# RL-VIG/LibContinual

Measured on AMD Instinct MI355X. Metric: images/sec/node (task-0 epoch), CIFAR-100 B50-5x10, higher is better.
Workload: dtype bf16; 1 GPU; lwf_resnet18_b50_task0; method=LWF, backbone=resnet18, per_gpu_batch=256, global_batch=256, image=3x32x32, parallelism=dp1, optimizer=fused SGD

## Files before the change

### include/clhip.h

```cpp
#ifndef CLHIP_H
#define CLHIP_H

#include <stddef.h>
#include <stdint.h>

#ifdef __cplusplus
extern "C" {
#endif

#define CLHIP_OK 0
#define CLHIP_EINVAL (-1)
#define CLHIP_EHIP (-2)
#define CLHIP_ENOMEM (-3)

#define CLHIP_BF16 0
#define CLHIP_F32 1

const char* clhip_last_error(void);
int clhip_version(void);

int clhip_nchw_to_nhwc(const float* x, void* y, int N, int C, int H, int W, int Cpad, int dtype, void* stream);
int clhip_nhwc_to_nchw(const void* y, float* x, int N, int C, int H, int W, int dtype, void* stream);

int clhip_conv_weight_prep(const float* w, void* w_fwd, void* w_dg, int K, int taps, int Creal, int Cpad,
// ... 19 lines not shown
                     int stride, int pad, int dtype, void* stream);

int clhip_bn_stats_finalize(const float* stat_partials, int tiles, int64_t M, int C, const float* gamma, const float* beta,
                            float* running_mean, float* running_var, float momentum, float eps, float* mean,
                            float* invstd, float* scale, float* shift, void* stream);
int clhip_bn_eval_affine(const float* gamma, const float* beta, const float* running_mean, const float* running_var,
                         float eps, int C, float* scale, float* shift, void* stream);
int clhip_bn_apply(const void* z, const float* scale, const float* shift, const void* res, void* y, int64_t M, int C,
                   int relu, int dtype, void* stream);
int clhip_bn_apply_eval(const void* z, const float* gamma, const float* beta, const float* running_mean, const float* running_var, float eps,
                        const void* res , void* y, int64_t M, int C, int relu, int dtype, void* stream);
int clhip_bn_apply_train(const void* z, const double* stat_acc, int replicas, int64_t M, int C, const float* gamma, const float* beta, float* rm,
                         float* rv, float momentum, float eps, float* mean, float* invstd, const void* res , void* y,
                         int relu, int dtype, void* stream);
int clhip_bn_apply_train_mask(const void* z, const double* stat_acc, int replicas, int64_t M, int C, const float* gamma, const float* beta, float* rm,
                              float* rv, float momentum, float eps, float* mean, float* invstd, const void* res , void* y,
                              void* relu_mask, int dtype, void* stream);
int clhip_bn_bwd_acc(const void* dy, const void* y, const void* z, const float* mean, const float* invstd, const float* gamma,
                     float* dgamma, float* dbeta, void* dz, void* dres, int dres_accumulate, int64_t M, int C, int relu, double* acc,
                     int replicas, int dtype, void* stream);
int clhip_bn_bwd_acc_zmask(const void* dy, const void* z, const float* mean, const float* invstd, const float* gamma, const float* beta,
                           float* dgamma, float* dbeta, void* dz, int64_t M, int C, double* acc, int replicas, int dtype, void* stream);
int clhip_bn_bwd_apply_acc(const void* dy, const void* y , const void* z, const float* mean, const float* invstd, const float* gamma,
                           const float* beta , float* dgamma, float* dbeta, void* dz, void* dres , int dres_accumulate,
                           int64_t M, int C, int relu, const double* acc, int replicas, int dtype, void* stream);
int clhip_bn_bwd_blocks(int64_t M, int C);
size_t clhip_bn_bwd_ws_floats(int64_t M, int C);
int clhip_bn_bwd(const void* dy, const void* y, const void* z, const float* mean, const float* invstd, const float* gamma,
                 float* dgamma, float* dbeta, void* dz, void* dres, int dres_accumulate, int64_t M, int C, int relu,
                 float* ws, int dtype, void* stream);

int clhip_avgpool_fwd(const void* a, float* feat, int N, int HW, int C, int dtype, void* stream);
int clhip_avgpool_bwd(const float* dfeat, void* da, int N, int HW, int C, int dtype, void* stream);
int clhip_avgpool_bwd_bn_reduce_supported(int N, int HW, int C, int dtype);
int clhip_avgpool_bwd_bn_reduce(const float* dfeat, void* da, const void* z_prod, const void* y_prod , const float* mean, const float* invstd,
                                double* acc, int replicas, int N, int HW, int C, int dtype, void* stream);

int clhip_maxpool_out_dim(int H);
int clhip_bn_relu_maxpool_fwd(const void* z, const double* stat_acc, int replicas, const float* gamma, const float* beta, float* running_mean,
                              float* running_var, float momentum, float eps, float* mean, float* invstd, void* y, void* argmax , int N, int H,
                              int W, int C, int training, int dtype, void* stream);
int clhip_maxpool_bwd_bn_reduce(const void* dy, const void* argmax, const void* z, const float* mean, const float* invstd, const float* gamma,
                                const float* beta, void* g, double* acc, int replicas, int N, int H, int W, int C, int dtype, void* stream);

int clhip_avgpool_win_fwd(const void* a, float* feat, int N, int H, int W, int C, int win, int dtype, void* stream);
int clhip_avgpool_win_bwd(const float* dfeat, void* da, int N, int H, int W, int C, int win, int dtype, void* stream);

int clhip_add_stats_blocks(int64_t M, int C);
int clhip_add_stats(void* z, const void* r, double* stat_acc, int replicas, int64_t M, int C, int dtype, void* stream);
int clhip_add_inplace(void* a, const void* b, int64_t n, int dtype, void* stream);

enum {
    CLHIP_UNIT_RELU = 1,
    CLHIP_UNIT_PRE_RES = 2,
    CLHIP_UNIT_RAW_SRC = 4,
    CLHIP_UNIT_NO_BN = 8,
    CLHIP_UNIT_MAXPOOL = 16
};

typedef struct {
    int32_t cin, cout, ksize, stride, pad;
    int32_t src;
    int32_t res;
    int32_t relu;
    int64_t w_off;
    int64_t gamma_off;
    int64_t beta_off;
    int64_t rm_off;
    int64_t rv_off;
} clhip_unit_desc;

typedef struct clhip_plan clhip_plan;

clhip_plan* clhip_plan_create(const clhip_unit_desc* units , int n_units, int N, int H, int W, int Cin, int dtype);
clhip_plan* clhip_plan_create_ex(const clhip_unit_desc* units , int n_units, int N, int H, int W, int Cin, int dtype, int pool_win);
void clhip_plan_destroy(clhip_plan*);
size_t clhip_plan_workspace_bytes(const clhip_plan*);
size_t clhip_plan_shadow_bytes(const clhip_plan*);
int clhip_plan_feat_dim(const clhip_plan*);
int clhip_plan_stage_status(clhip_plan*);
long long clhip_plan_stage_info(const clhip_plan*, int what);
int clhip_plan_stage_trace(clhip_plan*, unsigned long long* out24);
int clhip_plan_prep_weights(clhip_plan*, const float* params, void* shadow, void* stream);
int clhip_plan_forward(clhip_plan*, const float* x, const float* params, float* bn_stats, const void* shadow,
                       void* workspace, float* feat, int training, void* stream);
int clhip_plan_forward_ex(clhip_plan*, const float* x, const float* params, float* bn_stats, const void* shadow,
                          void* workspace, float* feat, int training, int64_t* num_batches_tracked, void* stream);
int clhip_plan_backward(clhip_plan*, const float* dfeat, const float* params, const void* shadow, void* workspace,
                        float* grads, void* stream);
int clhip_plan_num_units(const clhip_plan* p);
int clhip_plan_backward_range(clhip_plan* p, const float* dfeat, const float* params, const void* shadow, void* workspace,
                              float* grads, int unit_hi, int unit_lo, void* stream);
int clhip_plan_read_act(clhip_plan*, const void* workspace, int idx, int which, float* out_nchw, void* stream);

int clhip_linear_fwd(const float* x, const float* w, const float* b , float* out, int B, int D, int O, void* stream);
int clhip_linear_bwd(const float* x, const float* w, const float* dout, float* dx , float* dw, float* db ,
                     int B, int D, int O, int accumulate, void* stream);
int clhip_ce_slice(const float* logits, const int64_t* labels, int B, int O, int lo, int hi, int pred_hi, float weight,
                   float* loss_out, int loss_accumulate, float* dlogits , int grad_accumulate,
                   int64_t* pred , int32_t* correct , void* stream);
int clhip_ce_window(const float* logits, const int64_t* labels, int B, int O, int lo, int hi, int pred_lo, int pred_hi, float weight,
                    float* loss_out, int loss_accumulate, float* dlogits , int grad_accumulate,
                    int64_t* pred , int32_t* correct , void* stream);
int clhip_kd_loss(const float* pred, int pred_stride, const float* soft, int soft_stride, int B, int k, float T,
                  float weight, float* loss_out, int loss_accumulate, float* dpred , int grad_accumulate,
                  void* stream);

int clhip_cosine_linear_fwd(const float* x, const float* w, float* out, float* xnorm, float* wnorm, int B, int D, int O, void* stream);
int clhip_cosine_linear_bwd(const float* x, const float* w, const float* out, const float* xnorm, const float* wnorm,
                            const float* dout, float* dx, float* dw, int B, int D, int O, int accumulate, void* stream);
int clhip_cos_embed_loss(const float* a, const float* b, int B, int D, float weight, float* loss_out, int loss_accumulate,
                         float* da, int grad_accumulate, void* stream);
int clhip_margin_rank_loss(const float* scores, const int64_t* labels, int B, int O, int num_old, int K, float margin,
                           float weight, float* loss_out, int loss_accumulate, float* dscores, int grad_accumulate,
                           int32_t* hard_count, void* stream);

int clhip_ewc_penalty(const float* p, const float* ref, const float* fisher, int64_t n, float weight, float* loss_out,
                      int loss_accumulate, void* stream);
int clhip_ewc_grad(const float* p, const float* ref, const float* fisher, float* g, int64_t n, float weight,
                   const float* dev_scale, void* stream);
int clhip_ewc_penalty_multi(int count, const float* const* p, const float* const* ref, const float* const* fisher, const int64_t* n, float weight,
                            float* loss_out, int loss_accumulate, void* stream);
int clhip_ewc_grad_multi(int count, const float* const* p, const float* const* ref, const float* const* fisher, float* const* g, const int64_t* n,
                         float weight, const float* dev_scale, void* stream);
int clhip_fisher_accum(float* fisher, const float* g, int64_t n, float scale, void* stream);
int clhip_fisher_merge(float* new_f, const float* old_f, int64_t n, float alpha, void* stream);
int clhip_sgd_step(float* p, const float* g, float* mom, int64_t n, float lr, float momentum, float weight_decay,
                   float grad_scale, const float* ewc_ref, const float* ewc_fisher, float ewc_weight, void* stream);
int clhip_sgd_step_multi(int count, float* const* p, const float* const* g, float* const* mom , const int64_t* n, float lr, float momentum,
                         float weight_decay, float grad_scale, void* stream);
int clhip_sgd_step_multi_zero(int count, float* const* p, float* const* g, float* const* mom , const int64_t* n, float lr, float momentum,
                              float weight_decay, float grad_scale, unsigned zero_grad_mask, void* stream);
int clhip_adam_step(float* p, const float* g, float* m, float* v, int64_t n, float lr, float beta1, float beta2, float eps,
                    float weight_decay, float grad_scale, int step, void* stream);
int clhip_sq_norm(const float* g, int64_t n, float* out, int accumulate, void* stream);
int clhip_scale(float* g, int64_t n, float s, void* stream);
int clhip_scale_dev(const float* g, float* out, int64_t n, float s, const float* dev_scale, void* stream);
int clhip_sigma_scale_fwd(const float* scores, const float* sigma_dev, float* logits, int64_t n, void* stream);
int clhip_sigma_scale_bwd(const float* scores, const float* sigma_dev, const float* dlogits, float* dscores, float* dsigma,
                          int dsigma_accumulate, int64_t n, void* stream);

int clhip_l2_normalize_rows(const float* x, float* out, int R, int D, void* stream);
int clhip_ncm_classify(const float* feats, const float* means, int B, int M, int D, int64_t* pred, void* stream);
int clhip_herding_select(const float* feats , int n, int D, int m, int32_t* chosen ,
                         float* ws , void* stream);
int clhip_herding_select_batched(const float* feats, const int32_t* offsets, int n_classes, int max_rows, int D, int m, int32_t* chosen, float* ws,
                                 void* stream);

int clhip_gemm_nt(const void* A, const void* B, void* C, const float* bias, const void* R, void* H, int M, int N, int K,
                  int lda, int ldb, int ldc, int ldr, int ldh, int epilogue, int dtype, void* stream);
int clhip_conv_dgrad_wgrad_supported(int N, int H, int W, int C, int Creal, int K, int ksize, int stride, int pad, int dtype);
int clhip_conv_dgrad_wgrad(const void* x, const void* dz, const void* w_dg, void* dx, int accumulate, float* dw, void* ws,
                           const void* z_prod, const void* y_prod, const float* mean, const float* invstd, double* acc, int replicas,
                           int N, int H, int W, int C, int Creal, int K, int ksize, int stride, int pad, int dtype, void* stream);

typedef struct clhip_bn_input {
    const double* stat_acc; int replicas;
    const float* gamma; const float* beta;
    float* running_mean; float* running_var;
    float momentum, eps;
    float* mean; float* invstd;
    float* coef;
} clhip_bn_input;
typedef struct clhip_bn_grad {
    const void* dy; const void* z;
    const double* sums; int replicas;
// ... 119 lines not shown
```

### libcontinual_amd/_lib.py

```python
import ctypes as C
import os
import re
import subprocess

_HERE = os.path.dirname(os.path.abspath(__file__))
LIB_PATH = os.path.join(_HERE, "libclhip.so")
HEADER_PATH = os.path.join(os.path.dirname(_HERE), "include", "clhip.h")

BF16, F32 = 0, 1


class ClhipError(RuntimeError):
    pass


class UnitDesc(C.Structure):
    _fields_ = [("cin", C.c_int32), ("cout", C.c_int32), ("ksize", C.c_int32), ("stride", C.c_int32), ("pad", C.c_int32),
                ("src", C.c_int32), ("res", C.c_int32), ("relu", C.c_int32),
                ("w_off", C.c_int64), ("gamma_off", C.c_int64), ("beta_off", C.c_int64),
                ("rm_off", C.c_int64), ("rv_off", C.c_int64)]


class VitDesc(C.Structure):
    _fields_ = [(n, C.c_int32) for n in ("img", "patch", "dim", "depth", "heads", "mlp", "lora_rank")] + [("block_ln_eps", C.c_float)]
# ... 6 lines not shown

class VitParams(C.Structure):
    _fields_ = [(n, C.c_void_p) for n in ("cls_token", "pos_embed", "pe_w", "pe_b", "norm_w", "norm_b")] + [("layers", C.POINTER(VitLayerParams))]


def build(force=False):
    script = os.path.join(_HERE, "csrc", "build.sh")
    if force:
        import shutil
        shutil.rmtree(os.path.join(_HERE, "csrc", "obj"), ignore_errors=True)
    subprocess.run(["bash", script], check=True)


_lib = None
_p, _i, _l, _f, _sz = C.c_void_p, C.c_int, C.c_int64, C.c_float, C.c_size_t

_PROTOS = {
    "clhip_last_error": (C.c_char_p, []),
    "clhip_version": (_i, []),
    "clhip_nchw_to_nhwc": (_i, [_p, _p, _i, _i, _i, _i, _i, _i, _p]),
    "clhip_nhwc_to_nchw": (_i, [_p, _p, _i, _i, _i, _i, _i, _p]),
    "clhip_conv_weight_prep": (_i, [_p, _p, _p, _i, _i, _i, _i, _i, _p]),
    "clhip_conv_fwd_tiles": (_i, [_i] * 8),
    "clhip_conv_fwd": (_i, [_p, _p, _p, _p] + [_i] * 9 + [_p]),
    "clhip_conv_fwd_acc": (_i, [_p, _p, _p, _p] + [_i] * 10 + [_p]),
    "clhip_bn_apply_train": (_i, [_p, _p, _i, _l, _i, _p, _p, _p, _p, _f, _f, _p, _p, _p, _p, _i, _i, _p]),
    "clhip_bn_apply_train_mask": (_i, [_p, _p, _i, _l, _i, _p, _p, _p, _p, _f, _f, _p, _p, _p, _p, _p, _i, _p]),
    "clhip_bn_bwd_acc": (_i, [_p, _p, _p, _p, _p, _p, _p, _p, _p, _p, _i, _l, _i, _i, _p, _i, _i, _p]),
    "clhip_bn_bwd_acc_zmask": (_i, [_p, _p, _p, _p, _p, _p, _p, _p, _p, _l, _i, _p, _i, _i, _p]),
    "clhip_conv_dgrad": (_i, [_p, _p, _p, _i] + [_i] * 9 + [_p]),
    "clhip_maxpool_out_dim": (_i, [_i]),
    "clhip_bn_relu_maxpool_fwd": (_i, [_p, _p, _i, _p, _p, _p, _p, _f, _f, _p, _p, _p, _p, _i, _i, _i, _i, _i, _i, _p]),
    "clhip_maxpool_bwd_bn_reduce": (_i, [_p, _p, _p, _p, _p, _p, _p, _p, _p, _i, _i, _i, _i, _i, _i, _p]),
    "clhip_conv_dgrad_bn_reduce_supported": (_i, [_i] * 9),
    "clhip_conv_dgrad_bn_reduce": (_i, [_p, _p, _p, _i, _p, _p, _p, _p, _p, _i] + [_i] * 9 + [_p]),
    "clhip_conv_dgrad_bn_reduce_overlapped": (_i, [_i] * 9),
    "clhip_conv_dgrad_bn_reduce_ex": (_i, [_p, _p, _p, _i, _p, _p, _p, _p, _p, _p, _p, _p, _i] + [_i] * 9 + [_p]),
    "clhip_bn_bwd_apply_acc": (_i, [_p, _p, _p, _p, _p, _p, _p, _p, _p, _p, _p, _i, _l, _i, _i, _p, _i, _i, _p]),
    "clhip_conv_wgrad_ws_bytes": (_sz, [_i] * 10),
    "clhip_conv_dgrad_wgrad_supported": (_i, [_i] * 10),
    "clhip_conv_bn_input_supported": (_i, [_i] * 9),
    "clhip_conv_fwd_acc_bn_input": (_i, [_p, _p, _p, _p, _p, _i] + [_i] * 9 + [_p]),
    "clhip_conv_fwd_acc_bn_res_input": (_i, [_p, _p, _p, _p, _p, _p, _i] + [_i] * 9 + [_p]),
    "clhip_conv_dgrad_wgrad_bn_input": (_i, [_p, _p, _p, _p, _p, _i, _p, _p, _p, _p, _p, _i] + [_i] * 10 + [_p]),
    "clhip_conv_dgrad_wgrad_bn_grad": (_i, [_p, _p, _p, _p, _p, _i, _p, _p, _p, _p, _p, _p, _p, _i] + [_i] * 10 + [_p]),
    "clhip_conv_dgrad_pair_supported": (_i, [_i] * 6),
    "clhip_conv_dgrad_pair_packed_bytes": (_sz, [_i, _i]),
    "clhip_conv_dgrad_pair_pack": (_i, [_p, _p, _p, _i, _i, _i, _p]),
    "clhip_conv_dgrad_pair": (_i, [_p, _p, _p, _p, _i] + [_i] * 6 + [_p]),
    "clhip_conv_dgrad_pair_bn_reduce_supported": (_i, [_i] * 6),
    "clhip_conv_dgrad_pair_bn_reduce": (_i, [_p, _p, _p, _p, _i, _p, _p, _p, _p, _p, _i] + [_i] * 6 + [_p]),
    "clhip_conv_wgrad_pair_supported": (_i, [_i] * 6),
    "clhip_conv_fwd_acc_pair_supported": (_i, [_i] * 6),
    "clhip_conv_fwd_acc_pair": (_i, [_p, _p, _p, _p, _p, _p, _i, _p, _i] + [_i] * 6 + [_p]),
    "clhip_conv_wgrad_pair": (_i, [_p] * 7 + [_i] * 6 + [_p]),
    "clhip_conv_dgrad_wgrad": (_i, [_p, _p, _p, _p, _i, _p, _p, _p, _p, _p, _p, _p, _i] + [_i] * 10 + [_p]),
    "clhip_conv_wgrad": (_i, [_p, _p, _p, _p] + [_i] * 10 + [_p]),
    "clhip_bn_stats_finalize": (_i, [_p, _i, _l, _i, _p, _p, _p, _p, _f, _f, _p, _p, _p, _p, _p]),
    "clhip_bn_eval_affine": (_i, [_p, _p, _p, _p, _f, _i, _p, _p, _p]),
    "clhip_bn_apply": (_i, [_p, _p, _p, _p, _p, _l, _i, _i, _i, _p]),
    "clhip_bn_apply_eval": (_i, [_p, _p, _p, _p, _p, _f, _p, _p, _l, _i, _i, _i, _p]),
    "clhip_bn_bwd_blocks": (_i, [_l, _i]),
    "clhip_bn_bwd_ws_floats": (_sz, [_l, _i]),
    "clhip_bn_bwd": (_i, [_p, _p, _p, _p, _p, _p, _p, _p, _p, _p, _i, _l, _i, _i, _p, _i, _p]),
    "clhip_avgpool_fwd": (_i, [_p, _p, _i, _i, _i, _i, _p]),
    "clhip_avgpool_bwd": (_i, [_p, _p, _i, _i, _i, _i, _p]),
    "clhip_avgpool_bwd_bn_reduce_supported": (_i, [_i] * 4),
    "clhip_avgpool_bwd_bn_reduce": (_i, [_p, _p, _p, _p, _p, _p, _p, _i, _i, _i, _i, _i, _p]),
    "clhip_avgpool_win_fwd": (_i, [_p, _p, _i, _i, _i, _i, _i, _i, _p]),
    "clhip_avgpool_win_bwd": (_i, [_p, _p, _i, _i, _i, _i, _i, _i, _p]),
    "clhip_add_stats_blocks": (_i, [_l, _i]),
    "clhip_add_stats": (_i, [_p, _p, _p, _i, _l, _i, _i, _p]),
    "clhip_add_inplace": (_i, [_p, _p, _l, _i, _p]),
    "clhip_plan_create": (_p, [C.POINTER(UnitDesc), _i, _i, _i, _i, _i, _i]),
    "clhip_plan_create_ex": (_p, [C.POINTER(UnitDesc), _i, _i, _i, _i, _i, _i, _i]),
    "clhip_plan_destroy": (None, [_p]),
    "clhip_plan_workspace_bytes": (_sz, [_p]),
    "clhip_plan_shadow_bytes": (_sz, [_p]),
    "clhip_plan_feat_dim": (_i, [_p]),
    "clhip_plan_stage_status": (_i, [_p]),
    "clhip_plan_stage_info": (C.c_longlong, [_p, _i]),
    "clhip_plan_stage_trace": (_i, [_p, _p]),
    "clhip_plan_prep_weights": (_i, [_p, _p, _p, _p]),
    "clhip_plan_forward": (_i, [_p, _p, _p, _p, _p, _p, _p, _i, _p]),
    "clhip_plan_forward_ex": (_i, [_p, _p, _p, _p, _p, _p, _p, _i, _p, _p]),
    "clhip_plan_backward": (_i, [_p, _p, _p, _p, _p, _p, _p]),
    "clhip_plan_num_units": (_i, [_p]),
    "clhip_plan_backward_range": (_i, [_p, _p, _p, _p, _p, _p, _i, _i, _p]),
    "clhip_plan_read_act": (_i, [_p, _p, _i, _i, _p, _p]),
    "clhip_linear_fwd": (_i, [_p, _p, _p, _p, _i, _i, _i, _p]),
    "clhip_linear_bwd": (_i, [_p, _p, _p, _p, _p, _p, _i, _i, _i, _i, _p]),
    "clhip_ce_slice": (_i, [_p, _p, _i, _i, _i, _i, _i, _f, _p, _i, _p, _i, _p, _p, _p]),
    "clhip_ce_window": (_i, [_p, _p, _i, _i, _i, _i, _i, _i, _f, _p, _i, _p, _i, _p, _p, _p]),
    "clhip_kd_loss": (_i, [_p, _i, _p, _i, _i, _i, _f, _f, _p, _i, _p, _i, _p]),
    "clhip_cosine_linear_fwd": (_i, [_p, _p, _p, _p, _p, _i, _i, _i, _p]),
    "clhip_cosine_linear_bwd": (_i, [_p, _p, _p, _p, _p, _p, _p, _p, _i, _i, _i, _i, _p]),
    "clhip_cos_embed_loss": (_i, [_p, _p, _i, _i, _f, _p, _i, _p, _i, _p]),
    "clhip_margin_rank_loss": (_i, [_p, _p, _i, _i, _i, _i, _f, _f, _p, _i, _p, _i, _p, _p]),
    "clhip_ewc_penalty": (_i, [_p, _p, _p, _l, _f, _p, _i, _p]),
    "clhip_ewc_grad": (_i, [_p, _p, _p, _p, _l, _f, _p, _p]),
    "clhip_ewc_penalty_multi": (_i, [_i, _p, _p, _p, _p, _f, _p, _i, _p]),
    "clhip_ewc_grad_multi": (_i, [_i, _p, _p, _p, _p, _p, _f, _p, _p]),
    "clhip_fisher_accum": (_i, [_p, _p, _l, _f, _p]),
    "clhip_fisher_merge": (_i, [_p, _p, _l, _f, _p]),
    "clhip_sgd_step": (_i, [_p, _p, _p, _l, _f, _f, _f, _f, _p, _p, _f, _p]),
    "clhip_sgd_step_multi": (_i, [_i, _p, _p, _p, _p, _f, _f, _f, _f, _p]),
    "clhip_sgd_step_multi_zero": (_i, [_i, _p, _p, _p, _p, _f, _f, _f, _f, C.c_uint, _p]),
    "clhip_adam_step": (_i, [_p, _p, _p, _p, _l, _f, _f, _f, _f, _f, _f, _i, _p]),
    "clhip_sq_norm": (_i, [_p, _l, _p, _i, _p]),
    "clhip_scale": (_i, [_p, _l, _f, _p]),
    "clhip_scale_dev": (_i, [_p, _p, _l, _f, _p, _p]),
    "clhip_sigma_scale_fwd": (_i, [_p, _p, _p, _l, _p]),
    "clhip_sigma_scale_bwd": (_i, [_p, _p, _p, _p, _p, _i, _l, _p]),
    "clhip_l2_normalize_rows": (_i, [_p, _p, _i, _i, _p]),
    "clhip_ncm_classify": (_i, [_p, _p, _i, _i, _i, _p, _p]),
    "clhip_herding_select": (_i, [_p, _i, _i, _i, _p, _p, _p]),
    "clhip_herding_select_batched": (_i, [_p, _p, _i, _i, _i, _i, _p, _p, _p]),
    "clhip_augment_crop_flip": (_i, [_p, _p, _p, _p, _p, _i, _i, _i, _i, _i, C.POINTER(C.c_float), C.POINTER(C.c_float), _p]),
    "clhip_augment_rrc_flip": (_i, [_p, _p, _p, _p, _i, _i, _i, _i, C.POINTER(C.c_float), C.POINTER(C.c_float), _p]),
    "clhip_augment_rrc_aa_ws_bytes": (_sz, [_i, _i, _i]),
    "clhip_augment_rrc_aa": (_i, [_p, _p, _p, _p, _p, _p, _p, _i, _i, _i, _i, _i, C.POINTER(C.c_float), C.POINTER(C.c_float), _p]),
    "clhip_gemm_nt": (_i, [_p, _p, _p, _p, _p, _p] + [_i] * 10 + [_p]),
    "clhip_config": (_i, [C.c_char_p, C.c_char_p]),
    "clhip_config_get": (C.c_char_p, [C.c_char_p]),
    "clhip_conv_bn_input_wt_supported": (_i, [_i] * 9),
    "clhip_conv_fwd_acc_bn_input_wt": (_i, [_p, _p, _p, _p, _p, _p, _i] + [_i] * 9 + [_p]),
    "clhip_gram_accum_batched": (_i, [_p, C.c_size_t, _i, _p, _i, _i, _i, _p]),
    "clhip_gemm8_config": (None, [_i]),
    "clhip_wgrad4_config": (None, [_i]),
    "clhip_attn_fwd": (_i, [_p, _p, _p, _i, _i, _i, _i, _i, _p]),
    "clhip_attn_bwd": (_i, [_p, _p, _p, _p, _p, _p, _i, _i, _i, _i, _i, _p]),
    "clhip_ln_fwd": (_i, [_p, _p, _p, _p, _p, _p, _i, _i, _f, _i, _p]),
    "clhip_ln_bwd": (_i, [_p, _p, _p, _p, _p, _p, _i, _i, _i, _p]),
    "clhip_ln_pool_fwd": (_i, [_p, _p, _p, _p, _i, _i, _i, _i, _f, _i, _p]),
    "clhip_ln_pool_bwd": (_i, [_p, _p, _p, _p, _i, _i, _i, _i, _f, _i, _p]),
    "clhip_patchify": (_i, [_p, _p, _i, _i, _i, _i, _p]),
    "clhip_vit_assemble": (_i, [_p, _p, _p, _p, _p, _i, _i, _i, _i, _i, _p]),
    "clhip_vit_prompt_grad": (_i, [_p, _p, _i, _i, _i, _i, _i, _p]),
    "clhip_weight_prep2": (_i, [_p, _p, _p, _i, _i, _p, _p, _p, _p, _i, _i, _p]),
    "clhip_lora_qkv_refresh": (_i, [_i, _p, _p, _p, _p, _p, _p, _p, _i, _i, _i, _p]),
    "clhip_lora_merge": (_i, [_p, _p, _p, _p, _p, _i, _i, _p]),
    "clhip_lora_grad_ws_bytes": (_sz, [_i, _i, _i]),
    "clhip_lora_acat": (_i, [_p, _p, _p, _i, _i, _i, _p]),
    "clhip_lora_grad": (_i, [_p, _p, _p, _p, _p, _p, _p, _p, _i, _i, _i, _i, _p]),
    "clhip_gram_accum": (_i, [_p, _p, _i, _i, _i, _p]),
    "clhip_l2p_select": (_i, [_p, _p, _p, _i, _i, _i, _i, _i, _p, _p, _p, _p, _p, _p]),
    "clhip_l2p_scatter": (_i, [_p, _p, _p, _i, _i, _i, _i, _p]),
    "clhip_vit_create": (_p, [C.POINTER(VitDesc), _i]),
    "clhip_vit_destroy": (None, [_p]),
    "clhip_vit_shadow_bytes": (_sz, [_p]),
    "clhip_vit_workspace_bytes": (_sz, [_p, _i, _i, _i]),
    "clhip_vit_prep_weights": (_i, [_p, C.POINTER(VitParams), _p, _i, _i, _p]),
    "clhip_vit_forward": (_i, [_p, C.POINTER(VitParams), _p, _p, _p, _i, _p, _i, _i, _p, _p, _p]),
    "clhip_vit_backward": (_i, [_p, C.POINTER(VitParams), _p, _p, _p, _p, C.POINTER(C.c_void_p), _p]),
    "clhip_vit_read_act": (_i, [_p, _p, _i, _i, _p, _p]),
}

_CHECKED = {}


def header_symbols():
    with open(HEADER_PATH) as f:
        src = f.read()
    src = re.sub(r"/\*.*?\*/", "", src, flags=re.S)
    return sorted(set(re.findall(r"\b(clhip_[a-z0-9_]+)\s*\(", src)))

# ... 35 lines not shown
```

### libcontinual_amd/csrc/api.hip

```cpp
#include <map>
#include <utility>
#include <vector>
#include <mutex>
#include <string>
#include <string.h>
#include <stdio.h>
#include <stdlib.h>

#include "common.h"

static thread_local char g_err[512] = "";

void clhip_set_error(const char* fmt, ...) {
    va_list ap;
    va_start(ap, fmt);
    vsnprintf(g_err, sizeof(g_err), fmt, ap);
    va_end(ap);
}

extern "C" const char* clhip_last_error(void) { return g_err; }
extern "C" int clhip_version(void) { return 103; }

namespace {
const char* const kKeys[] = {
    "ATTN_GENERIC", "ATTN_BWD", "BN_FUSE", "BN_FUSE_MAX_M", "BN_MASK_BITS", "BN_MASK_FROM_Y", "BN_PARTIALS", "CE_ROWS", "CE_ONE_WG", "LINEAR_BWD_SPLIT", "CONV3G", "CONV4", "CONV_V1",
    "GEMM_NO_SPLIT", "GEMM_TAIL", "NO_CONV16", "NO_CONV3", "NO_PARITY_DGRAD", "NO_SHORTCUT", "NO_STEM", "PREP_NARROW", "WGRAD4",
    "WGRAD_NO_TR", "WGRAD2_ATOMIC", "WGRAD_DEFER", "WGRAD_DEFER_SIDE", "BWD_FUSED", "WGRAD_STREAM", "BRANCH_STREAM", "WGRAD_ALWAYS_QUEUE", "SIDE_PRIO", "EVENT_FLAGS", "EVENT_RECORD", "CONV5", "CONV6", "WGRAD16_PARTS", "WGRAD32_IPG", "WGRAD64_IPG", "WGRAD64_IPI2", "CONV64", "CONV64_BM", "CONV64_FWD", "CONV6_PAIR", "CONV7", "CONV7_TPW", "WGRAD7", "FWD7", "PAIR_BN_FUSE", "POOL_BN_FUSE", "BN_INPUT", "BN_INPUT_WT", "BN_RES_INPUT", "BN_GRAD", "BN_GRAD_MINC", "BN_GRAD_RES", "CONV6_DEBUG", "BN_ONEPASS", "WGRAD5", "WGRAD32",
    "BN_ACC_CPT", "BN_BWD_ITERS", "CONV3_CFG", "CONV4_CFG", "CONV4_GRID", "GEMM_GROUP_M", "GEMM_MT", "IGEMM_TILE",
    "SHORTCUT_MIN_PIXELS", "STEM_GRID", "STEM_WGRAD_GRID", "WGRAD4_MIN_STEPS", "WGRAD4_MIN_TOTAL", "WGRAD_NET_GFLOP", "WGRAD_TARGET",
    "CONV5_MIN_TILES", "CONV5_GRID", "CONV64_MAX_W", "CONV64_MAX_M", "CONV8", "CONV8_MIN_TILES", "DZ_BUFFERS", "CONV8_GRID", "CONV8_OPT", "CONV8_BNR", "CONV9", "PLAN_SKIP", "WT_DEBUG", "EVAL_LAZY", "GEMM_SPLITK", "STREAM_PROBE", "STAGE_EVAL", "STAGE_TRAIN", "STAGE_TRAIN_BWD", "STAGE_TRACE", "STAGE_ENTRY", "STAGE_ENTRY_BWD", "STAGE_POOL", "STAGE_XCH3",
    "CONV3_DEBUG", "WGRAD_DEBUG", "CONV4_FORCE_CFG", "CONV4_ENABLE", "CONV4_DEBUG", "CONV4_TRACE", "WGRAD4_TRACE", "CONV6_TRACE", "CONV8_TRACE", "CONV9_TRACE",
};
std::mutex g_stream_mu;
std::mutex g_cfg_mu;
std::map<std::string, const char*>& cfg_map() { static std::map<std::string, const char*> m; return m; }
bool known_key(const char* k) {
    for (const char* q : kKeys) if (strcmp(q, k) == 0) return true;
    return false;
}
}

namespace {
__global__ void stream_probe_spin_kernel(unsigned long long* out, long long ticks) {
    const unsigned long long t0 = wall_clock64();
    while ((long long)(wall_clock64() - t0) < ticks) __builtin_amdgcn_s_sleep(64);
    out[0] = wall_clock64();
}
__global__ void stream_probe_stamp_kernel(unsigned long long* out) { out[1] = wall_clock64(); }

struct SharedStreams {
    std::vector<hipStream_t> pool;
    std::map<std::pair<hipStream_t, int>, hipStream_t> chosen;
    hipStream_t low_prio = nullptr;
    unsigned long long* probe_buf = nullptr;
};
SharedStreams g_shared[16];

bool runs_beside(SharedStreams& S, hipStream_t a, hipStream_t b) {
    if (S.probe_buf == nullptr && hipMalloc(reinterpret_cast<void**>(&S.probe_buf), 2 * sizeof(unsigned long long)) != hipSuccess) return false;
    hipLaunchKernelGGL(stream_probe_spin_kernel, dim3(1), dim3(1), 0, a, S.probe_buf, 30000ll);
    hipLaunchKernelGGL(stream_probe_stamp_kernel, dim3(1), dim3(1), 0, b, S.probe_buf);
    if (hipStreamSynchronize(b) != hipSuccess || hipStreamSynchronize(a) != hipSuccess) return false;
    unsigned long long h[2] = {0, 0};
    if (hipMemcpy(h, S.probe_buf, sizeof(h), hipMemcpyDeviceToHost) != hipSuccess) return false;
    return h[1] < h[0];
}
}

hipStream_t clhip_shared_stream(int role, hipStream_t main_s, bool low_priority) {
    int dev = 0;
    if (hipGetDevice(&dev) != hipSuccess || dev < 0 || dev >= 16 || role < 0 || role > 1) return nullptr;
    std::lock_guard<std::mutex> lk(g_stream_mu);
    SharedStreams& S = g_shared[dev];
    if (low_priority) {
        if (S.low_prio == nullptr) {
            int prio_lo = 0, prio_hi = 0;
            (void)hipDeviceGetStreamPriorityRange(&prio_lo, &prio_hi);
            if (hipStreamCreateWithPriority(&S.low_prio, hipStreamNonBlocking, prio_lo) != hipSuccess) S.low_prio = nullptr;
        }
        return S.low_prio;
    }
    (void)role;
    const auto key = std::make_pair(main_s, 0);
    auto it = S.chosen.find(key);
    if (it != S.chosen.end()) return it->second;
    {
        hipStreamCaptureStatus cap = hipStreamCaptureStatusNone;
        (void)hipStreamIsCapturing(main_s, &cap);
        if (cap != hipStreamCaptureStatusNone) {
            for (const auto& kv : S.chosen) if (kv.second != main_s) return kv.second;
            for (hipStream_t c : S.pool) if (c != main_s) return c;
            return nullptr;
        }
    }
    const int probe_cfg = clhip_cfg("STREAM_PROBE") != nullptr ? atoi(clhip_cfg("STREAM_PROBE")) : 1;
    hipStream_t pick = nullptr, fallback = nullptr;
    for (size_t k = 0; k < 8 && pick == nullptr; ++k) {
        if (k == S.pool.size()) {
            hipStream_t s = nullptr;
            if (hipStreamCreateWithFlags(&s, hipStreamNonBlocking) != hipSuccess) break;
            S.pool.push_back(s);
        }
        hipStream_t c = S.pool[k];
        if (c == main_s) continue;
        if (fallback == nullptr) fallback = c;
        if (probe_cfg == 0 || runs_beside(S, main_s, c)) pick = c;
    }
    if (pick == nullptr) pick = fallback;
    if (pick != nullptr) S.chosen[key] = pick;
    return pick;
}

// ... 72 lines not shown
```

### libcontinual_amd/csrc/common.h

```cpp
#pragma once
#include <hip/hip_runtime.h>
#include <stdint.h>
#include <stdio.h>
#include <stdarg.h>

#include "../../include/clhip.h"

typedef uint16_t bf16_t;
typedef __attribute__((ext_vector_type(8))) __bf16 bf16x8_t;
typedef __attribute__((ext_vector_type(4))) float f32x4;
typedef __attribute__((ext_vector_type(4))) short s16x4;

void clhip_set_error(const char* fmt, ...);
hipStream_t clhip_shared_stream(int role, hipStream_t main_s, bool low_priority);
const char* clhip_cfg(const char* name);

#define CLHIP_CHECK_ARG(cond)                                                          \
    do {                                                                               \
        if (!(cond)) {                                                                 \
            clhip_set_error("%s:%d: invalid argument: %s", __FILE__, __LINE__, #cond); \
            return CLHIP_EINVAL;                                                       \
        }                                                                              \
    } while (0)

#define CLHIP_LAUNCH_CHECK()                                                                          \
    do {                                                                                              \
        hipError_t e_ = hipGetLastError();                                                            \
        if (e_ != hipSuccess) {                                                                       \
            clhip_set_error("%s:%d: kernel launch failed: %s", __FILE__, __LINE__, hipGetErrorString(e_)); \
            return CLHIP_EHIP;                                                                        \
        }                                                                                             \
    } while (0)

__device__ __forceinline__ float bf16_to_f32(bf16_t v) { return __uint_as_float(((uint32_t)v) << 16); }
__device__ __forceinline__ bf16_t f32_to_bf16(float f) {
    uint32_t u = __float_as_uint(f);
    if ((u & 0x7fffffffu) > 0x7f800000u) return (bf16_t)((u >> 16) | 0x40);
    u += 0x7fffu + ((u >> 16) & 1u);
    return (bf16_t)(u >> 16);
}

typedef __attribute__((ext_vector_type(2))) float f32x2_t;
typedef __attribute__((ext_vector_type(2))) __bf16 bf16x2_t;
__device__ __forceinline__ uint32_t pack_bf16x2(float lo, float hi) {
    f32x2_t v = {lo, hi};
    return __builtin_bit_cast(uint32_t, __builtin_convertvector(v, bf16x2_t));
}

template <typename T> struct Elem;
template <> struct Elem<bf16_t> {
    static constexpr int DTYPE = CLHIP_BF16;
    __device__ static __forceinline__ float ld(const bf16_t* p) { return bf16_to_f32(*p); }
    __device__ static __forceinline__ void st(bf16_t* p, float v) { *p = f32_to_bf16(v); }
};
template <> struct Elem<float> {
    static constexpr int DTYPE = CLHIP_F32;
    __device__ static __forceinline__ float ld(const float* p) { return *p; }
    __device__ static __forceinline__ void st(float* p, float v) { *p = v; }
};

template <typename T> __device__ __forceinline__ void load8(const T* p, float (&v)[8]);
template <> __device__ __forceinline__ void load8<bf16_t>(const bf16_t* p, float (&v)[8]) {
    uint4 u = *reinterpret_cast<const uint4*>(p);
    uint32_t w[4] = {u.x, u.y, u.z, u.w};
#pragma unroll
    for (int i = 0; i < 4; ++i) {
        v[2 * i] = __uint_as_float(w[i] << 16);
        v[2 * i + 1] = __uint_as_float(w[i] & 0xffff0000u);
    }
}
template <> __device__ __forceinline__ void load8<float>(const float* p, float (&v)[8]) {
    float4 a = *reinterpret_cast<const float4*>(p);
    float4 b = *reinterpret_cast<const float4*>(p + 4);
    v[0] = a.x; v[1] = a.y; v[2] = a.z; v[3] = a.w; v[4] = b.x; v[5] = b.y; v[6] = b.z; v[7] = b.w;
}
template <typename T> __device__ __forceinline__ void store8(T* p, const float (&v)[8]);
template <> __device__ __forceinline__ void store8<bf16_t>(bf16_t* p, const float (&v)[8]) {
    *reinterpret_cast<uint4*>(p) = make_uint4(pack_bf16x2(v[0], v[1]), pack_bf16x2(v[2], v[3]), pack_bf16x2(v[4], v[5]), pack_bf16x2(v[6], v[7]));
}
template <> __device__ __forceinline__ void store8<float>(float* p, const float (&v)[8]) {
    *reinterpret_cast<float4*>(p) = make_float4(v[0], v[1], v[2], v[3]);
    *reinterpret_cast<float4*>(p + 4) = make_float4(v[4], v[5], v[6], v[7]);
}

__device__ __forceinline__ void unpack8(uint4 u, float (&v)[8]) {
    const uint32_t w[4] = {u.x, u.y, u.z, u.w};
#pragma unroll
    for (int i = 0; i < 4; ++i) {
        v[2 * i] = __uint_as_float(w[i] << 16);
        v[2 * i + 1] = __uint_as_float(w[i] & 0xffff0000u);
    }
}

__device__ __forceinline__ float wave_sum(float v) {
#pragma unroll
    for (int o = 32; o > 0; o >>= 1) v += __shfl_xor(v, o, 64);
    return v;
}
__device__ __forceinline__ float wave_max(float v) {
#pragma unroll
    for (int o = 32; o > 0; o >>= 1) v = fmaxf(v, __shfl_xor(v, o, 64));
    return v;
}

__device__ __forceinline__ float block_sum_256(float v, float* red) {
    v = wave_sum(v);
    __syncthreads();
    if ((threadIdx.x & 63) == 0) red[threadIdx.x >> 6] = v;
    __syncthreads();
    return red[0] + red[1] + red[2] + red[3];
}

static inline int ilog2_exact(int v) {
    if (v <= 0 || (v & (v - 1))) return -1;
    int l = 0;
    while ((1 << l) < v) ++l;
    return l;
}
static inline int64_t cdiv64(int64_t a, int64_t b) { return (a + b - 1) / b; }

__device__ __forceinline__ float row16_sum(float v) {
    v += __builtin_bit_cast(float, __builtin_amdgcn_update_dpp(0, __builtin_bit_cast(int, v), 0xB1, 0xF, 0xF, true));
    v += __builtin_bit_cast(float, __builtin_amdgcn_update_dpp(0, __builtin_bit_cast(int, v), 0x4E, 0xF, 0xF, true));
    v += __builtin_bit_cast(float, __builtin_amdgcn_update_dpp(0, __builtin_bit_cast(int, v), 0x141, 0xF, 0xF, true));
    v += __builtin_bit_cast(float, __builtin_amdgcn_update_dpp(0, __builtin_bit_cast(int, v), 0x140, 0xF, 0xF, true));
    return v;
}

template <int N>
// ... 129 lines not shown
```

### libcontinual_amd/csrc/elementwise.hip

```cpp
#include "common.h"

namespace {

int ew_blocks4(int64_t n4) {
    int64_t b = (n4 + 255) / 256;
    if (b > 2048) b = 2048;
    if (b < 1) b = 1;
    return (int)b;
}

__global__ __launch_bounds__(256) void ewc_penalty_kernel(const float* __restrict__ p, const float* __restrict__ ref,
                                                          const float* __restrict__ f, int64_t n, int64_t n4, float weight,
                                                          float* out) {
    __shared__ float red[4];
    float acc = 0.f;
    const int64_t stride = (int64_t)gridDim.x * blockDim.x;
    for (int64_t i = (int64_t)blockIdx.x * blockDim.x + threadIdx.x; i < n4; i += stride) {
        float4 a = reinterpret_cast<const float4*>(p)[i], b = reinterpret_cast<const float4*>(ref)[i],
               c = reinterpret_cast<const float4*>(f)[i];
        float d0 = a.x - b.x, d1 = a.y - b.y, d2 = a.z - b.z, d3 = a.w - b.w;
        acc += c.x * d0 * d0 + c.y * d1 * d1 + c.z * d2 * d2 + c.w * d3 * d3;
    }
    for (int64_t i = (n4 << 2) + (int64_t)blockIdx.x * blockDim.x + threadIdx.x; i < n; i += stride) {
        float d = p[i] - ref[i];
// ... 7 lines not shown
                                                       const float* __restrict__ f, float* __restrict__ g, int64_t n, float weight,
                                                       const float* __restrict__ dev_scale) {
    if (dev_scale != nullptr) weight *= *dev_scale;
    const int64_t stride = (int64_t)gridDim.x * blockDim.x;
    for (int64_t i = (int64_t)blockIdx.x * blockDim.x + threadIdx.x; i < n; i += stride) g[i] += weight * f[i] * (p[i] - ref[i]);
}

constexpr int kEwcSegs = 4;
struct EwcSeg { const float* p; const float* ref; const float* f; float* g; long long n, n4; unsigned first_block, blocks; };
struct EwcTable { int n; EwcSeg s[kEwcSegs]; };

__global__ __launch_bounds__(256) void ewc_penalty_multi_kernel(EwcTable t, float weight, float* out) {
    __shared__ float red[4];
    int u = 0;
    while (u + 1 < t.n && blockIdx.x >= t.s[u + 1].first_block) ++u;
    const EwcSeg& e = t.s[u];
    const long long stride = (long long)e.blocks * 256;
    const long long i0 = (long long)(blockIdx.x - e.first_block) * 256 + threadIdx.x;
    float acc = 0.f;
    for (long long i = i0; i < e.n4; i += stride) {
        float4 a = reinterpret_cast<const float4*>(e.p)[i], b = reinterpret_cast<const float4*>(e.ref)[i], c = reinterpret_cast<const float4*>(e.f)[i];
        float d0 = a.x - b.x, d1 = a.y - b.y, d2 = a.z - b.z, d3 = a.w - b.w;
        acc += c.x * d0 * d0 + c.y * d1 * d1 + c.z * d2 * d2 + c.w * d3 * d3;
    }
    for (long long i = (e.n4 << 2) + i0; i < e.n; i += stride) {
        float d = e.p[i] - e.ref[i];
        acc += e.f[i] * d * d;
    }
    float s = block_sum_256(acc, red);
    if (threadIdx.x == 0) atomicAdd(out, 0.5f * weight * s);
}

__global__ __launch_bounds__(256) void ewc_grad_multi_kernel(EwcTable t, float weight, const float* __restrict__ dev_scale) {
    if (dev_scale != nullptr) weight *= *dev_scale;
    int u = 0;
    while (u + 1 < t.n && blockIdx.x >= t.s[u + 1].first_block) ++u;
    const EwcSeg& e = t.s[u];
    const long long stride = (long long)e.blocks * 256;
    for (long long i = (long long)(blockIdx.x - e.first_block) * 256 + threadIdx.x; i < e.n; i += stride) e.g[i] += weight * e.f[i] * (e.p[i] - e.ref[i]);
}

__global__ __launch_bounds__(256) void fisher_accum_kernel(float* __restrict__ fi, const float* __restrict__ g, int64_t n, float scale) {
    const int64_t stride = (int64_t)gridDim.x * blockDim.x;
    for (int64_t i = (int64_t)blockIdx.x * blockDim.x + threadIdx.x; i < n; i += stride) {
        float v = g[i];
        fi[i] += v * v * scale;
    }
}

__global__ __launch_bounds__(256) void fisher_merge_kernel(float* __restrict__ nf, const float* __restrict__ of, int64_t n, float alpha) {
    const int64_t stride = (int64_t)gridDim.x * blockDim.x;
    for (int64_t i = (int64_t)blockIdx.x * blockDim.x + threadIdx.x; i < n; i += stride) nf[i] = alpha * of[i] + (1.f - alpha) * nf[i];
}

template <bool MOM, bool EWC>
__global__ __launch_bounds__(256) void sgd_kernel(float* __restrict__ p, const float* __restrict__ g, float* __restrict__ m, int64_t n,
                                                  float lr, float momentum, float wd, float gscale, const float* __restrict__ ref,
                                                  const float* __restrict__ fi, float ew) {
    const int64_t stride = (int64_t)gridDim.x * blockDim.x;
    for (int64_t i = (int64_t)blockIdx.x * blockDim.x + threadIdx.x; i < n; i += stride) {
        float pv = p[i];
        float d = g[i] * gscale;
        if (EWC) d += ew * fi[i] * (pv - ref[i]);
        d = fmaf(wd, pv, d);
        if (MOM) {
            float b = fmaf(momentum, m[i], d);
            m[i] = b;
            d = b;
        }
        p[i] = fmaf(-lr, d, pv);
    }
}

constexpr int kSgdSegs = 8;
struct SgdSeg { float* p; float* g; float* m; long long n; unsigned first_block, blocks; int zero; };
struct SgdTable { int n; SgdSeg s[kSgdSegs]; };
template <bool MOM>
__global__ __launch_bounds__(256) void sgd_multi_kernel(SgdTable t, float lr, float momentum, float wd, float gscale) {
    int u = 0;
    while (u + 1 < t.n && blockIdx.x >= t.s[u + 1].first_block) ++u;
    const SgdSeg& e = t.s[u];
    const long long stride = (long long)e.blocks * 256;
    for (long long i = (long long)(blockIdx.x - e.first_block) * 256 + threadIdx.x; i < e.n; i += stride) {
        float pv = e.p[i];
        float d = e.g[i] * gscale;
        d = fmaf(wd, pv, d);
        if (MOM) {
            float b = fmaf(momentum, e.m[i], d);
            e.m[i] = b;
            d = b;
        }
        e.p[i] = fmaf(-lr, d, pv);
        if (e.zero) e.g[i] = 0.f;
    }
}

__global__ __launch_bounds__(256) void adam_kernel(float* __restrict__ p, const float* __restrict__ g, float* __restrict__ m,
                                                   float* __restrict__ v, int64_t n, float lr, float b1, float b2, float eps, float wd,
                                                   float gscale, float bc1, float bc2s) {
    const int64_t stride = (int64_t)gridDim.x * blockDim.x;
    for (int64_t i = (int64_t)blockIdx.x * blockDim.x + threadIdx.x; i < n; i += stride) {
        float pv = p[i];
        float d = fmaf(wd, pv, g[i] * gscale);
        float mi = b1 * m[i] + (1.f - b1) * d;
        float vi = b2 * v[i] + (1.f - b2) * d * d;
        m[i] = mi; v[i] = vi;
        float denom = sqrtf(vi) / bc2s + eps;
        p[i] = pv - (lr / bc1) * (mi / denom);
    }
}

__global__ __launch_bounds__(256) void sq_norm_kernel(const float* __restrict__ g, int64_t n, float* out) {
    __shared__ float red[4];
    float acc = 0.f;
    const int64_t stride = (int64_t)gridDim.x * blockDim.x;
    for (int64_t i = (int64_t)blockIdx.x * blockDim.x + threadIdx.x; i < n; i += stride) acc += g[i] * g[i];
    float s = block_sum_256(acc, red);
    if (threadIdx.x == 0) atomicAdd(out, s);
}

__global__ __launch_bounds__(256) void scale_kernel(float* __restrict__ g, int64_t n, float s) {
    const int64_t stride = (int64_t)gridDim.x * blockDim.x;
    for (int64_t i = (int64_t)blockIdx.x * blockDim.x + threadIdx.x; i < n; i += stride) g[i] *= s;
}

__global__ __launch_bounds__(256) void scale_dev_kernel(const float* __restrict__ g, float* __restrict__ out, int64_t n, float s,
                                                        const float* __restrict__ dev_scale) {
    if (dev_scale != nullptr) s *= *dev_scale;
    const int64_t stride = (int64_t)gridDim.x * blockDim.x;
    for (int64_t i = (int64_t)blockIdx.x * blockDim.x + threadIdx.x; i < n; i += stride) out[i] = g[i] * s;
}

__global__ __launch_bounds__(256) void sigma_fwd_kernel(const float* __restrict__ sc, const float* __restrict__ sigma, float* __restrict__ out,
                                                        int64_t n) {
    const float s = *sigma;
    const int64_t stride = (int64_t)gridDim.x * blockDim.x;
    for (int64_t i = (int64_t)blockIdx.x * blockDim.x + threadIdx.x; i < n; i += stride) out[i] = sc[i] * s;
}

__global__ __launch_bounds__(256) void sigma_bwd_kernel(const float* __restrict__ sc, const float* __restrict__ sigma,
                                                        const float* __restrict__ dl, float* __restrict__ dsc, float* dsigma, int64_t n) {
    __shared__ float red[4];
    const float s = *sigma;
    float acc = 0.f;
    const int64_t stride = (int64_t)gridDim.x * blockDim.x;
    for (int64_t i = (int64_t)blockIdx.x * blockDim.x + threadIdx.x; i < n; i += stride) {
        float d = dl[i];
        acc = fmaf(d, sc[i], acc);
        if (dsc != nullptr) dsc[i] = d * s;
    }
    float t = block_sum_256(acc, red);
    if (threadIdx.x == 0 && dsigma != nullptr) atomicAdd(dsigma, t);
}

}

extern "C" int clhip_ewc_penalty(const float* p, const float* ref, const float* fisher, int64_t n, float weight, float* loss_out,
                                 int loss_accumulate, void* stream) {
    CLHIP_CHECK_ARG(p && ref && fisher && loss_out && n >= 0);
    hipStream_t st = (hipStream_t)stream;
    if (!loss_accumulate) {
        if (hipMemsetAsync(loss_out, 0, sizeof(float), st) != hipSuccess) { clhip_set_error("memset failed"); return CLHIP_EHIP; }
    }
    if (n == 0) return CLHIP_OK;
    bool aligned = (((uintptr_t)p | (uintptr_t)ref | (uintptr_t)fisher) & 15) == 0;
    int64_t n4 = aligned ? (n >> 2) : 0;
    hipLaunchKernelGGL(ewc_penalty_kernel, dim3(ew_blocks4(aligned ? (n >> 2) + 1 : n)), dim3(256), 0, st, p, ref, fisher, n, n4,
                       weight, loss_out);
    CLHIP_LAUNCH_CHECK();
    return CLHIP_OK;
}

static int ewc_table(int count, const float* const* p, const float* const* ref, const float* const* fisher, float* const* g, const int64_t* n, bool vec4,
                     EwcTable& t, unsigned& blocks) {
    t.n = 0; blocks = 0;
// ... 168 lines not shown
```

### libcontinual_amd/csrc/plan.hip

```cpp
#include <stdlib.h>
#include <vector>
#include <new>

#include "common.h"

void clhip_bn_set_stop_event(hipEvent_t ev);
hipEvent_t clhip_bn_pending_stop_event();
void clhip_bn_set_fwd_stop_event(hipEvent_t ev);
void clhip_wgrad_defer_begin();
int clhip_wgrad_defer_flush(hipStream_t st, bool end);
void clhip_wgrad_defer_abort();
void clhip_wgrad_defer_pause(bool paused);

namespace {
constexpr float kBnMomentum = 0.1f;
constexpr float kBnEps = 1e-5f;

size_t align_up(size_t v, size_t a = 256) { return (v + a - 1) / a * a; }

struct Act {
    int H, W, C;
    size_t y_off;
    size_t dy_off;
    size_t bytes;
// ... 24 lines not shown
    int64_t M;
    int tiles;
    size_t z_off;
    size_t sh_fwd, sh_dg;
    size_t sh_pk;
    int pair;
    int lazy_to;
    int lazy_from;
    int res_lazy_to;
    int res_lazy_from;
    int wt_to;
    int wt_from;
    bool pair_fuse_bn;
    bool fpair;
    bool wpair;
    bool pair_acc;
    size_t f_mean, f_invstd, f_scale, f_shift;
    size_t a_fwd, a_bwd;
    int rep_fwd, rep_bwd;
    int dx_acc, dres_acc;
    bool relu, pre_res, raw_src, no_bn;
    bool maxpool;
    size_t am_off, pg_off;
    bool has_dzr;
    size_t dzr_off;
    size_t mask_off;
    int branch;
    int forks;
    int joins;
    size_t wg_own;
    int stage_len;
    int entry_first;
    int run_first;
    size_t st_slab;
    bool stage_train;
    bool fuse_src_bn;
};
}

struct clhip_plan {
    int N, H, W, Cin, Cin_pad, dtype, esize;
    std::vector<Unit> units;
    std::vector<Act> acts;
    size_t ws_bytes, shadow_bytes;
    size_t dz_off;
    static constexpr int kDz = 4;
    size_t dz_offs[kDz];
    int n_dz;
    size_t dz_off2;
    hipStream_t side;
    hipEvent_t ev_dz[kDz], ev_wg[kDz], ev_end;
    bool wg_pending[kDz];
    static constexpr int kMaxBranch = 8;
    hipStream_t br;
    hipEvent_t ev_fork[kMaxBranch], ev_join[kMaxBranch], ev_bfork[kMaxBranch], ev_bjoin[kMaxBranch];
    int n_branch;
    int br_act;
    int br_slot;
    hipEvent_t ev_br_end;
    hipEvent_t bfork_ev[kMaxBranch];
    size_t wg_off2;
    bool defer_reduce;
    int defer_side;
    size_t f_base;
    size_t f_part, f_bnws;
    size_t wg_off;
    size_t acc_off, acc_bytes;
    bool use_acc;
    std::vector<char> res_pending;
    std::vector<char> wt_pending;
    const float* params_dev = nullptr;
    const float* bn_stats_dev = nullptr;
    std::vector<char> stage_skipped;
    std::vector<char> eval_unwritten;
    std::vector<char> lazy_live;
    std::vector<char> bwd_sums_ready;
    std::vector<char> mask_stale;
    void* xch = nullptr;
    hipStream_t xch_stream = nullptr;
    bool xch_used = false;
    long long st_fwd_launches = 0, st_bwd_launches = 0;
    int feat_dim;
    bool side_ok;
    int pool_win;
};

extern "C" clhip_plan* clhip_plan_create(const clhip_unit_desc* units, int n_units, int N, int H, int W, int Cin, int dtype) {
    return clhip_plan_create_ex(units, n_units, N, H, W, Cin, dtype, 0);
}

extern "C" clhip_plan* clhip_plan_create_ex(const clhip_unit_desc* units, int n_units, int N, int H, int W, int Cin, int dtype, int pool_win) {
    if (!units || n_units <= 0 || N <= 0 || H <= 0 || W <= 0 || Cin <= 0 || pool_win < 0 || (dtype != CLHIP_BF16 && dtype != CLHIP_F32)) {
        clhip_set_error("clhip_plan_create: invalid argument");
        return nullptr;
    }
    clhip_plan* p = new (std::nothrow) clhip_plan();
    if (!p) { clhip_set_error("out of host memory"); return nullptr; }
    p->N = N; p->H = H; p->W = W; p->Cin = Cin; p->dtype = dtype; p->esize = dtype == CLHIP_BF16 ? 2 : 4;
    p->pool_win = pool_win;
    p->Cin_pad = (Cin + 7) / 8 * 8;
    if (ilog2_exact(p->Cin_pad) < 0) { int c = 8; while (c < Cin) c <<= 1; p->Cin_pad = c; }
    size_t off = 0, sh = 0;
    Act a0{H, W, p->Cin_pad, 0, 0, (size_t)N * H * W * p->Cin_pad * p->esize};
    a0.y_off = off; off = align_up(off + a0.bytes);
    p->acts.push_back(a0);
    size_t max_z = 0, max_part = 0, max_bnws = 0, nfloat = 0, max_wg = 0, ndouble = 0;
    const bool want_acc = clhip_cfg("BN_PARTIALS") == nullptr;
    auto replicas = [](int producers) { int r = 1; while (r < 32 && producers > 64 * r) r <<= 1; return r; };
    p->use_acc = false;
    for (int i = 0; i < n_units; ++i) {
        Unit u{};
        u.d = units[i];
        u.relu = (u.d.relu & CLHIP_UNIT_RELU) != 0; u.pre_res = (u.d.relu & CLHIP_UNIT_PRE_RES) != 0;
        u.raw_src = (u.d.relu & CLHIP_UNIT_RAW_SRC) != 0; u.no_bn = (u.d.relu & CLHIP_UNIT_NO_BN) != 0;
        u.maxpool = (u.d.relu & CLHIP_UNIT_MAXPOOL) != 0;
        const bool stem7 = u.d.ksize == 7 && u.maxpool && i == 0 && u.d.src == 0 && p->Cin_pad == 8 && u.d.stride == 2 && u.d.pad == 3;
        if (u.d.src < 0 || u.d.src > i || u.d.res > i || (u.d.ksize != 1 && u.d.ksize != 3 && !stem7) || u.d.stride < 1 || u.d.cout % 16 ||
            (u.raw_src && u.d.src < 1) || (u.pre_res && u.d.res < 1) || (u.no_bn && (u.pre_res || u.relu || u.d.res >= 0)) ||
            (u.maxpool && (i != 0 || u.d.src != 0 || !u.relu || u.d.res >= 0 || u.pre_res || u.raw_src || u.no_bn)) ||
            (u.d.relu & ~(CLHIP_UNIT_RELU | CLHIP_UNIT_PRE_RES | CLHIP_UNIT_RAW_SRC | CLHIP_UNIT_NO_BN | CLHIP_UNIT_MAXPOOL))) {
            clhip_set_error("clhip_plan_create: bad unit %d", i);
            delete p;
            return nullptr;
        }
        const Act& s = p->acts[u.d.src];
        u.cin_pad = s.C;
        if ((u.d.src == 0 && u.d.cin != Cin) || (u.d.src != 0 && u.d.cin != s.C)) {
            clhip_set_error("clhip_plan_create: unit %d channel mismatch", i);
            delete p;
            return nullptr;
        }
        u.H = s.H; u.W = s.W;
        u.Ho = (s.H + 2 * u.d.pad - u.d.ksize) / u.d.stride + 1;
        u.Wo = (s.W + 2 * u.d.pad - u.d.ksize) / u.d.stride + 1;
        u.M = (int64_t)N * u.Ho * u.Wo;
        u.tiles = clhip_conv_fwd_tiles(N, u.H, u.W, u.cin_pad, u.d.cout, u.d.ksize, u.d.stride, u.d.pad);
        if (u.d.res >= 0) {
            const Act& r = p->acts[u.d.res];
            if (r.H != u.Ho || r.W != u.Wo || r.C != u.d.cout) {
                clhip_set_error("clhip_plan_create: unit %d residual shape mismatch", i);
                delete p;
                return nullptr;
            }
        }
        size_t bytes = (size_t)u.M * u.d.cout * p->esize;
        u.z_off = off; off = align_up(off + bytes);
        if (u.maxpool) {
            const int Hp = clhip_maxpool_out_dim(u.Ho), Wp = clhip_maxpool_out_dim(u.Wo);
            const size_t pooled = (size_t)N * Hp * Wp * u.d.cout;
            Act a{Hp, Wp, u.d.cout, off, 0, pooled * p->esize};
            off = align_up(off + a.bytes);
            p->acts.push_back(a);
            u.am_off = off; off = align_up(off + pooled);
            u.pg_off = off; off = align_up(off + bytes);
        } else {
            Act a{u.Ho, u.Wo, u.d.cout, off, 0, bytes};
            off = align_up(off + bytes);
            p->acts.push_back(a);
        }
        size_t wbytes = (size_t)u.d.cout * u.d.ksize * u.d.ksize * u.cin_pad * p->esize;
        u.sh_fwd = sh; sh = align_up(sh + wbytes);
        u.sh_dg = sh; sh = align_up(sh + wbytes);
        u.f_mean = nfloat; u.f_invstd = nfloat + u.d.cout; u.f_scale = nfloat + 2 * (size_t)u.d.cout; u.f_shift = nfloat + 3 * (size_t)u.d.cout;
        nfloat += 4 * (size_t)u.d.cout;
        const bool pow2 = (u.d.cout & (u.d.cout - 1)) == 0;
        u.rep_fwd = (want_acc && pow2) ? replicas(u.tiles) : 0;
        if (u.pre_res) {
            if (!pow2) { clhip_set_error("clhip_plan_create: unit %d: a pre-BatchNorm residual needs a power-of-two channel count", i); delete p; return nullptr; }
            u.rep_fwd = replicas(clhip_add_stats_blocks(u.M, u.d.cout));
        }
        u.rep_bwd = (want_acc && pow2) ? replicas(clhip_bn_bwd_blocks(u.M, u.d.cout)) : 0;
        static const bool mask_bits = !(clhip_cfg("BN_MASK_BITS") && atoi(clhip_cfg("BN_MASK_BITS")) == 0);
        u.mask_off = 0;
        if (mask_bits && u.relu && u.d.res >= 0 && !u.pre_res && !u.no_bn && !u.raw_src && u.rep_fwd > 0 && u.rep_bwd > 0) {
            u.mask_off = off;
            off = align_up(off + (size_t)u.M * u.d.cout / 8);
        }
        if (u.no_bn) u.rep_fwd = u.rep_bwd = 0;
        if (u.maxpool && (u.rep_fwd <= 0 || u.rep_bwd <= 0)) {
            clhip_set_error("clhip_plan_create: unit %d: the max-pool stem needs the BatchNorm accumulator path (CLHIP_BN_PARTIALS unset)", i);
            delete p;
            return nullptr;
        }
        u.a_fwd = ndouble; ndouble += 2 * (size_t)u.d.cout * (u.rep_fwd > 0 ? u.rep_fwd : 1);
        u.a_bwd = ndouble; ndouble += 2 * (size_t)u.d.cout * (u.rep_bwd > 0 ? u.rep_bwd : 1);
        if (u.rep_fwd || u.rep_bwd) p->use_acc = true;
        if (bytes > max_z) max_z = bytes;
        size_t part = (size_t)u.tiles * 2 * u.d.cout;
        if (part > max_part) max_part = part;
        size_t bw = clhip_bn_bwd_ws_floats(u.M, u.d.cout);
        if (bw > max_bnws) max_bnws = bw;
        size_t wg = clhip_conv_wgrad_ws_bytes(N, u.H, u.W, u.cin_pad, u.d.cin, u.d.cout, u.d.ksize, u.d.stride, u.d.pad, dtype);
        if (wg > max_wg) max_wg = wg;
        p->units.push_back(u);
    }
    p->n_branch = 0; p->br = nullptr; p->br_act = -1; p->br_slot = -1;
    size_t max_wg2 = 0;
    for (auto& u : p->units) { u.branch = u.forks = u.joins = -1; }
    static const bool branch_off = clhip_cfg("BRANCH_STREAM") != nullptr && atoi(clhip_cfg("BRANCH_STREAM")) == 0;
    for (int b = 0; b < n_units && !branch_off; ++b) {
        Unit& u = p->units[b];
        if (u.d.ksize != 1 || u.relu || u.pre_res || u.raw_src || u.no_bn || u.d.res >= 0 || u.rep_fwd <= 0 || u.rep_bwd <= 0 || u.d.src < 1) continue;
        if (p->n_branch >= clhip_plan::kMaxBranch) break;
        int consumer = -1, n_cons = 0;
        for (int k = 0; k < n_units; ++k) {
            const Unit& o = p->units[k];
            if (o.d.src == b + 1) n_cons += 2;
            if (o.d.res == b + 1) { ++n_cons; consumer = k; }
        }
        if (n_cons != 1 || consumer <= b || p->units[consumer].pre_res || p->units[consumer].rep_fwd <= 0 || p->units[consumer].rep_bwd <= 0) continue;
        Unit& prod = p->units[u.d.src - 1];
        if (prod.no_bn || prod.maxpool || prod.rep_fwd <= 0 || prod.forks >= 0 || p->units[consumer].joins >= 0) continue;
        u.branch = p->n_branch; prod.forks = p->n_branch; p->units[consumer].joins = p->n_branch;
        ++p->n_branch;
        size_t wg = clhip_conv_wgrad_ws_bytes(N, u.H, u.W, u.cin_pad, u.d.cin, u.d.cout, u.d.ksize, u.d.stride, u.d.pad, dtype);
        if (wg > max_wg2) max_wg2 = wg;
    }
    for (size_t i = 1; i < p->acts.size(); ++i) { p->acts[i].dy_off = off; off = align_up(off + p->acts[i].bytes); }
    for (int i = 0; i < n_units; ++i) {
        const Unit& c = p->units[i];
        const int targets[2] = {c.pre_res ? c.d.res : 0, c.raw_src ? c.d.src : 0};
        for (int t : targets) {
            if (t < 1) continue;
            Unit& prod = p->units[t - 1];
            if (prod.has_dzr) { clhip_set_error("clhip_plan_create: the raw output of unit %d has two raw consumers", t - 1); delete p; return nullptr; }
            prod.has_dzr = true;
            prod.dzr_off = off; off = align_up(off + p->acts[t].bytes);
        }
    }
    for (int i = 0; i < n_units; ++i)
        if (p->units[i].no_bn && !p->units[i].has_dzr) { clhip_set_error("clhip_plan_create: unit %d has no BatchNorm and no consumer", i); delete p; return nullptr; }
    {
        const double net_flops = 1.0e9 * (clhip_cfg("WGRAD_NET_GFLOP") ? atof(clhip_cfg("WGRAD_NET_GFLOP")) : 4.0);
        p->side_ok = false;
        for (const Unit& u : p->units)
            if (2.0 * (double)u.M * u.d.ksize * u.d.ksize * u.d.cin * u.d.cout >= net_flops) p->side_ok = true;
    }
    p->dz_off = off; off = align_up(off + max_z);
    p->dz_off2 = off; off = align_up(off + max_z);
    {
        static const int ndz_cfg = clhip_cfg("DZ_BUFFERS") ? atoi(clhip_cfg("DZ_BUFFERS")) : clhip_plan::kDz;
        p->n_dz = (p->side_ok && ndz_cfg >= 2 && ndz_cfg <= clhip_plan::kDz) ? ndz_cfg : 2;
        p->dz_offs[0] = p->dz_off; p->dz_offs[1] = p->dz_off2;
        for (int q = 2; q < clhip_plan::kDz; ++q) {
            p->dz_offs[q] = p->dz_off;
            if (q < p->n_dz) { p->dz_offs[q] = off; off = align_up(off + max_z); }
        }
    }
    p->wg_off = off; off = align_up(off + max_wg);
    static const bool defer_off = clhip_cfg("WGRAD_DEFER") != nullptr && atoi(clhip_cfg("WGRAD_DEFER")) == 0;
    p->defer_reduce = !p->side_ok && !defer_off;
    static const int defer_side = clhip_cfg("WGRAD_DEFER_SIDE") ? atoi(clhip_cfg("WGRAD_DEFER_SIDE")) : 0;
    p->defer_side = p->side_ok ? defer_side : 0;
    for (Unit& u : p->units) {
        u.wg_own = p->wg_off;
        if (p->defer_reduce || p->defer_side > 0) {
            u.wg_own = off;
            off = align_up(off + clhip_conv_wgrad_ws_bytes(N, u.H, u.W, u.cin_pad, u.d.cin, u.d.cout, u.d.ksize, u.d.stride, u.d.pad, dtype));
        }
    }
    p->wg_off2 = off; off = align_up(off + max_wg2);
    p->f_base = off;
    nfloat = (nfloat + 63) / 64 * 64;
    p->f_part = nfloat; nfloat += (max_part + 63) / 64 * 64;
    p->f_bnws = nfloat; nfloat += (max_bnws + 63) / 64 * 64;
    off = align_up(off + nfloat * sizeof(float));
    p->acc_off = off; p->acc_bytes = ndouble * sizeof(double);
    off = align_up(off + p->acc_bytes);
    p->ws_bytes = off;
    p->shadow_bytes = sh;
    {
        const Act& last = p->acts.back();
        if (p->units.back().no_bn || (pool_win > 0 && (last.H < pool_win || last.W < pool_win))) {
            clhip_set_error("clhip_plan_create: the last unit cannot feed the pool");
            delete p;
            return nullptr;
        }
        p->feat_dim = pool_win > 0 ? last.C * (last.H / pool_win) * (last.W / pool_win) : last.C;
    }
    std::vector<char> written(p->acts.size(), 0);
    written.back() = 1;
    for (int i = n_units - 1; i >= 0; --i) {
        Unit& u = p->units[i];
        if (u.d.res >= 0 && !u.pre_res) { u.dres_acc = written[u.d.res]; written[u.d.res] = 1; }
        if (u.d.src != 0 && !u.raw_src) { u.dx_acc = written[u.d.src]; written[u.d.src] = 1; }
    }
    const char* fe = clhip_cfg("BN_FUSE");
    const bool fuse_on = fe == nullptr || atoi(fe) != 0;
    const long long fuse_max_m = clhip_cfg("BN_FUSE_MAX_M") ? atoll(clhip_cfg("BN_FUSE_MAX_M")) : ((fe == nullptr && p->side_ok) ? 16384 : (1ll << 62));
    p->bwd_sums_ready.assign(p->units.size(), 0);
    p->mask_stale.assign(p->units.size(), 0);
    for (int i = 0; i < n_units; ++i) {
        Unit& u = p->units[i];
        u.fuse_src_bn = false;
        if (!fuse_on || u.d.src < 1 || u.raw_src || u.pre_res || u.no_bn) continue;
        if ((long long)u.M > fuse_max_m && !clhip_conv_dgrad_bn_reduce_overlapped(N, u.H, u.W, u.cin_pad, u.d.cout, u.d.ksize, u.d.stride, u.d.pad, dtype)) continue;
        const int a = u.d.src;
        const Unit& prod = p->units[a - 1];
        if (prod.no_bn || prod.pre_res || prod.raw_src || prod.has_dzr || prod.rep_bwd <= 0 || prod.maxpool) continue;
        bool lowest = true;
        for (int k = 0; k < n_units; ++k) {
            if (k == i) continue;
            const Unit& o = p->units[k];
            const bool consumes = (o.d.src == a && !o.raw_src) || (o.d.res == a && !o.pre_res);
            if (consumes && k < i) lowest = false;
        }
        if (u.d.res == a) lowest = false;
        if (!lowest) continue;
        if (!clhip_conv_dgrad_bn_reduce_supported(N, u.H, u.W, u.cin_pad, u.d.cout, u.d.ksize, u.d.stride, u.d.pad, dtype)) continue;
        u.fuse_src_bn = true;
    }
    for (auto& u : p->units) { u.pair = -1; u.pair_acc = false; u.sh_pk = 0; u.wpair = u.fpair = u.pair_fuse_bn = false; }
    const char* pair_cfg = clhip_cfg("CONV6_PAIR");
    const bool pair_off = pair_cfg != nullptr && atoi(pair_cfg) == 0;
    for (int b = 0; b < n_units && !pair_off; ++b) {
        Unit& ub = p->units[b];
        if (ub.d.ksize != 1 || ub.d.stride != 2 || ub.d.pad != 0 || ub.pre_res || ub.raw_src || ub.no_bn || ub.has_dzr || ub.d.src < 1) continue;
        int a = -1, users = 0;
        for (int k = 0; k < n_units; ++k) {
            const Unit& o = p->units[k];
            if (o.d.src == ub.d.src || o.d.res == ub.d.src) ++users;
            if (k < b && o.d.src == ub.d.src && o.d.ksize == 3 && o.d.stride == 2 && o.d.pad == 1 && !o.raw_src && !o.pre_res && !o.no_bn && !o.has_dzr &&
                o.d.cout == ub.d.cout && o.cin_pad == ub.cin_pad && !o.fuse_src_bn)
                a = k;
        }
        if (a < 0 || users != 2 || p->units[a].pair >= 0) continue;
        Unit& ua = p->units[a];
        if (!clhip_conv_dgrad_pair_supported(N, ua.H, ua.W, ua.cin_pad, ua.d.cout, dtype)) continue;
        ua.pair = b; ub.pair = a;
        ua.pair_acc = ub.dx_acc;
        ua.sh_pk = p->shadow_bytes; p->shadow_bytes = align_up(p->shadow_bytes + clhip_conv_dgrad_pair_packed_bytes(ua.cin_pad, ua.d.cout));
        {
            const Unit& prod = p->units[ua.d.src - 1];
            ua.pair_fuse_bn = fuse_on && !prod.no_bn && !prod.maxpool && !prod.pre_res && !prod.raw_src && !prod.has_dzr && prod.rep_bwd > 0 && (long long)prod.M <= fuse_max_m &&
                              clhip_conv_dgrad_pair_bn_reduce_supported(N, ua.H, ua.W, ua.cin_pad, ua.d.cout, dtype) != 0;
        }
        ua.fpair = ub.fpair = ua.rep_fwd > 0 && ub.rep_fwd > 0 && ua.cin_pad == ua.d.cin &&
                              clhip_conv_fwd_acc_pair_supported(N, ua.H, ua.W, ua.cin_pad, ua.d.cout, dtype) != 0;
        ua.wpair = ub.wpair = p->defer_reduce && ua.cin_pad == ua.d.cin && ub.cin_pad == ub.d.cin &&
                              clhip_conv_wgrad_pair_supported(N, ua.H, ua.W, ua.cin_pad, ua.d.cout, dtype) != 0;
    }
    for (auto& u : p->units) { u.lazy_to = u.lazy_from = -1; }
    p->lazy_live.assign(p->units.size(), 0);
    p->eval_unwritten.assign(p->units.size(), 0);
// ... 244 lines not shown
struct PrepEntry { int64_t w_off; int64_t wf_off, wd_off; int64_t wp_off; int wp_tap0; int K, taps, Creal, Cpad; unsigned first_block; };
__device__ __forceinline__ size_t packed_index(int c, int tap, int k, int K, int Cpad) {
    if (Cpad < 64) return ((size_t)c * 10 + tap) * K + k;
    return ((((size_t)(c >> 6) * (K >> 4) + (k >> 4)) * 64 + (c & 63)) * 21 + tap * 2 + ((k >> 3) & 1)) * 8 + (k & 7);
}
struct PrepTable { int n; unsigned first[kPrepMax]; PrepEntry e[kPrepMax]; };
__device__ __forceinline__ int prep_entry_of_block(const PrepTable& t) {
    static_assert(kPrepMax <= 64, "one lane per entry");
    const int l = threadIdx.x & 63;
    const bool le = l < t.n && t.first[l < kPrepMax ? l : 0] <= blockIdx.x;
    return __popcll(__ballot(le)) - 1;
}

template <typename T>
__global__ __launch_bounds__(256) void weight_prep_multi_kernel(const float* __restrict__ params, char* __restrict__ shadow, PrepTable t) {
    __shared__ float tile[32][33];
    const int u = __builtin_amdgcn_readfirstlane(prep_entry_of_block(t));
    const PrepEntry& d = t.e[u];
    const int kb = (d.K + 31) / 32, cb = (d.Cpad + 31) / 32;
    int r = blockIdx.x - d.first_block;
    const int c0 = (r % cb) * 32; r /= cb;
    const int k0 = (r % kb) * 32;
    const int tap = r / kb;
    const int tx = threadIdx.x & 31, ty = threadIdx.x >> 5;
    T* wf = reinterpret_cast<T*>(shadow + d.wf_off);
    for (int i = ty; i < 32; i += 8) {
        const int k = k0 + i, c = c0 + tx;
        float v = 0.f;
        if (k < d.K && c < d.Cpad) {
            if (c < d.Creal) v = params[d.w_off + ((size_t)k * d.taps + tap) * d.Creal + c];
            Elem<T>::st(wf + ((size_t)k * d.taps + tap) * d.Cpad + c, v);
        }
        tile[i][tx] = v;
    }
    if (d.wd_off < 0) return;
    __syncthreads();
    T* wd = reinterpret_cast<T*>(shadow + d.wd_off);
    for (int i = ty; i < 32; i += 8) {
        const int c = c0 + i, k = k0 + tx;
        if (c < d.Cpad && k < d.K) {
            Elem<T>::st(wd + ((size_t)c * d.taps + tap) * d.K + k, tile[tx][i]);
            if (d.wp_off >= 0) Elem<T>::st(reinterpret_cast<T*>(shadow + d.wp_off) + packed_index(c, d.wp_tap0 + tap, k, d.K, d.Cpad), tile[tx][i]);
        }
    }
}

__global__ __launch_bounds__(256) void weight_prep_multi64_kernel(const float* __restrict__ params, char* __restrict__ shadow, PrepTable t) {
    __shared__ float tile[64][65];
    const int u = __builtin_amdgcn_readfirstlane(prep_entry_of_block(t));
    const PrepEntry& d = t.e[u];
    const int kb = (d.K + 63) / 64, cb = (d.Cpad + 63) / 64;
    int r = blockIdx.x - d.first_block;
    const int c0 = (r % cb) * 64; r /= cb;
    const int k0 = (r % kb) * 64;
    const int tap = r / kb;
    const int tx = (threadIdx.x & 15) * 4, ty = threadIdx.x >> 4;
    bf16_t* wf = reinterpret_cast<bf16_t*>(shadow + d.wf_off);
#pragma unroll
    for (int i = 0; i < 4; ++i) {
        const int kk = ty + 16 * i, k = k0 + kk, c = c0 + tx;
        float v[4] = {0.f, 0.f, 0.f, 0.f};
        if (k < d.K && c < d.Cpad) {
            const float* src = params + d.w_off + ((size_t)k * d.taps + tap) * d.Creal + c;
#pragma unroll
            for (int e = 0; e < 4; ++e) if (c + e < d.Creal) v[e] = src[e];
            *reinterpret_cast<uint2*>(wf + ((size_t)k * d.taps + tap) * d.Cpad + c) = make_uint2(pack_bf16x2(v[0], v[1]), pack_bf16x2(v[2], v[3]));
        }
#pragma unroll
        for (int e = 0; e < 4; ++e) tile[kk][tx + e] = v[e];
    }
    if (d.wd_off < 0) return;
    __syncthreads();
    bf16_t* wd = reinterpret_cast<bf16_t*>(shadow + d.wd_off);
#pragma unroll
    for (int i = 0; i < 4; ++i) {
        const int cc = ty + 16 * i, c = c0 + cc, k = k0 + tx;
        if (c < d.Cpad && k < d.K) {
            const uint2 v = make_uint2(pack_bf16x2(tile[tx][cc], tile[tx + 1][cc]), pack_bf16x2(tile[tx + 2][cc], tile[tx + 3][cc]));
            *reinterpret_cast<uint2*>(wd + ((size_t)c * d.taps + tap) * d.K + k) = v;
            if (d.wp_off >= 0) *reinterpret_cast<uint2*>(reinterpret_cast<bf16_t*>(shadow + d.wp_off) + packed_index(c, d.wp_tap0 + tap, k, d.K, d.Cpad)) = v;
        }
    }
}
}

extern "C" int clhip_plan_prep_weights(clhip_plan* p, const float* params, void* shadow, void* stream) {
    CLHIP_CHECK_ARG(p && params && shadow);
    char* sh = static_cast<char*>(shadow);
    size_t i = 0;
    while (i < p->units.size()) {
        PrepTable t;
        t.n = 0;
        unsigned blocks = 0;
        bool wide = p->dtype == CLHIP_BF16;
        static const bool no_wide = clhip_cfg("PREP_NARROW") != nullptr;
        for (size_t j = i; j < p->units.size() && j < i + kPrepMax; ++j)
            wide = wide && !no_wide && p->units[j].d.cout % 4 == 0 && p->units[j].cin_pad % 4 == 0 && p->units[j].sh_fwd % 8 == 0 && p->units[j].sh_dg % 8 == 0;
        const int tb = wide ? 64 : 32;
        for (; i < p->units.size() && t.n < kPrepMax; ++i) {
            const Unit& u = p->units[i];
            PrepEntry& e = t.e[t.n++];
            e.w_off = u.d.w_off; e.wf_off = (int64_t)u.sh_fwd; e.wd_off = u.d.src != 0 ? (int64_t)u.sh_dg : -1;
            e.wp_off = -1; e.wp_tap0 = 0;
            if (u.pair >= 0) {
                const bool owner = u.d.ksize == 3;
                e.wp_off = (int64_t)(owner ? u.sh_pk : p->units[u.pair].sh_pk);
                e.wp_tap0 = owner ? 0 : 9;
            }
            e.K = u.d.cout; e.taps = u.d.ksize * u.d.ksize; e.Creal = u.d.cin; e.Cpad = u.cin_pad;
            e.first_block = blocks; t.first[t.n - 1] = blocks;
            blocks += (unsigned)(e.taps * ((e.K + tb - 1) / tb) * ((e.Cpad + tb - 1) / tb));
        }
        if (wide) hipLaunchKernelGGL(weight_prep_multi64_kernel, dim3(blocks), dim3(256), 0, (hipStream_t)stream, params, sh, t);
        else if (p->dtype == CLHIP_BF16) hipLaunchKernelGGL(weight_prep_multi_kernel<bf16_t>, dim3(blocks), dim3(256), 0, (hipStream_t)stream, params, sh, t);
        else hipLaunchKernelGGL(weight_prep_multi_kernel<float>, dim3(blocks), dim3(256), 0, (hipStream_t)stream, params, sh, t);
        CLHIP_LAUNCH_CHECK();
    }
    return CLHIP_OK;
}

namespace {
template <typename T>
__global__ __launch_bounds__(256) void plan_prologue_kernel(const float* __restrict__ x, T* __restrict__ y, int N, int C, int HW, int Cpad, unsigned layout_blocks,
                                                            uint4* __restrict__ acc, size_t acc_n16, long long* __restrict__ nbt, unsigned long long nbt_mask_lo,
                                                            unsigned long long nbt_mask_hi, int n_units) {
    if (blockIdx.x >= layout_blocks) {
        const size_t i0 = (size_t)(blockIdx.x - layout_blocks) * 256 * 4 + threadIdx.x;
#pragma unroll
        for (int k = 0; k < 4; ++k) { const size_t i = i0 + (size_t)k * 256; if (i < acc_n16) acc[i] = make_uint4(0, 0, 0, 0); }
        return;
    }
    if (nbt != nullptr && blockIdx.x == 0)
        for (int u = threadIdx.x; u < n_units; u += 256)
            if ((u < 64 ? (nbt_mask_lo >> u) : (nbt_mask_hi >> (u - 64))) & 1ull) nbt[u] += 1;
    const int64_t pix = (int64_t)blockIdx.x * 256 + threadIdx.x;
    if (pix >= (int64_t)N * HW) return;
    const int n = (int)(pix / HW), hw = (int)(pix - (int64_t)n * HW);
    for (int c0 = 0; c0 < Cpad; c0 += 8) {
        float v[8];
#pragma unroll
        for (int e = 0; e < 8; ++e) v[e] = (c0 + e < C) ? x[((size_t)n * C + c0 + e) * HW + hw] : 0.f;
        store8<T>(y + pix * Cpad + c0, v);
    }
}
}

extern "C" int clhip_plan_forward(clhip_plan* p, const float* x, const float* params, float* bn_stats, const void* shadow,
                                  void* workspace, float* feat, int training, void* stream) {
    return clhip_plan_forward_ex(p, x, params, bn_stats, shadow, workspace, feat, training, nullptr, stream);
}

extern "C" int clhip_plan_forward_ex(clhip_plan* p, const float* x, const float* params, float* bn_stats, const void* shadow,
                                     void* workspace, float* feat, int training, int64_t* num_batches_tracked, void* stream) {
    CLHIP_CHECK_ARG(p && x && params && bn_stats && shadow && workspace && feat);
    CLHIP_CHECK_ARG(num_batches_tracked == nullptr || p->units.size() <= 128);
    char* ws = static_cast<char*>(workspace);
    const char* sh = static_cast<const char*>(shadow);
    float* fr = reinterpret_cast<float*>(ws + p->f_base);
    double* acc = reinterpret_cast<double*>(ws + p->acc_off);
    const bool use_acc = training && p->use_acc;
    std::fill(p->bwd_sums_ready.begin(), p->bwd_sums_ready.end(), 0);
    {
        const int64_t npix = (int64_t)p->N * p->H * p->W;
        const unsigned lb = (unsigned)((npix + 255) / 256);
        const size_t n16 = use_acc ? p->acc_bytes / 16 : 0;
        const unsigned ab = (unsigned)((n16 + 1023) / 1024);
        unsigned long long mlo = 0, mhi = 0;
        for (size_t i = 0; i < p->units.size() && i < 128; ++i)
            if (!p->units[i].no_bn) { if (i < 64) mlo |= 1ull << i; else mhi |= 1ull << (i - 64); }
        long long* nbt = training ? reinterpret_cast<long long*>(num_batches_tracked) : nullptr;
        uint4* a16 = reinterpret_cast<uint4*>(acc);
        if (p->dtype == CLHIP_BF16)
            hipLaunchKernelGGL(plan_prologue_kernel<bf16_t>, dim3(lb + ab), dim3(256), 0, (hipStream_t)stream, x, reinterpret_cast<bf16_t*>(ws + p->acts[0].y_off), p->N, p->Cin,
                               p->H * p->W, p->Cin_pad, lb, a16, n16, nbt, mlo, mhi, (int)p->units.size());
        else
            hipLaunchKernelGGL(plan_prologue_kernel<float>, dim3(lb + ab), dim3(256), 0, (hipStream_t)stream, x, reinterpret_cast<float*>(ws + p->acts[0].y_off), p->N, p->Cin,
                               p->H * p->W, p->Cin_pad, lb, a16, n16, nbt, mlo, mhi, (int)p->units.size());
        CLHIP_LAUNCH_CHECK();
    }
    const char* br_cfg_f = clhip_cfg("BRANCH_STREAM");
// ... 376 lines not shown
                        const Unit& uq = p->units[e0 + q];
                        const int blocks = q < 2 ? p->N : clhip_stage_train_slab_blocks(p->N, uq.d.cout);
                        TRY(clhip_wgrad_reduce_launch(reinterpret_cast<const float*>(ws + uq.st_slab), grads + uq.d.w_off, (int64_t)uq.d.cout * uq.d.ksize * uq.d.ksize * uq.cin_pad / 4,
                                                      blocks, main_s));
                    }
                    i = e0;
                    continue;
                }
                const void* wdv[16]; const float *gv[16], *bv[16], *mev[16], *isv[16]; const void *zv[16], *yv[16]; float *dgv[16], *dbv[16], *slv[16]; void* dzv[16];
                for (int q = 0; q < len; ++q) {
                    const Unit& uq = p->units[f + q];
                    wdv[q] = sh + uq.sh_dg; gv[q] = params + uq.d.gamma_off; bv[q] = params + uq.d.beta_off; mev[q] = fr + uq.f_mean; isv[q] = fr + uq.f_invstd;
                    zv[q] = ws + uq.z_off; yv[q] = (q & 1) ? ws + p->acts[f + q + 1].y_off : nullptr;
                    dgv[q] = grads + uq.d.gamma_off; dbv[q] = grads + uq.d.beta_off; slv[q] = reinterpret_cast<float*>(ws + uq.st_slab);
                    dzv[q] = ws + p->acts[f + q + 1].dy_off;
                }
                if (p->br_act >= 0) join_branch();
                TRY(stage_train_serialize(p, main_s));
                TRY(clhip_stage_train_bwd_launch(ws + p->acts[uf.d.src].y_off, ws + p->acts[f + len].dy_off, ws + p->acts[uf.d.src].dy_off, p->units[f + 1].dres_acc, p->N, uf.H,
                                                 uf.W, uf.d.cout, len, wdv, gv, bv, mev, isv, zv, yv, dgv, dbv, slv, dzv, p->xch, stage_trace_cfg(uf.d.cout), 0,
                                                 pool_in_stage && f + len == (int)p->units.size() ? dfeat : nullptr, p->dtype, main_s));
                ++p->st_bwd_launches;
                for (int q = len - 1; q >= 0; --q) {
                    const Unit& uq = p->units[f + q];
                    TRY(clhip_wgrad_reduce_launch(reinterpret_cast<const float*>(ws + uq.st_slab), grads + uq.d.w_off, (int64_t)uq.d.cout * 9 * uq.cin_pad / 4, clhip_stage_train_slab_blocks(p->N, uq.d.cout), main_s));
                }
                i = f;
                continue;
            }
        }
        const Unit& u = p->units[i];
        const Act& src = p->acts[u.d.src];
        const Act& dst = p->acts[i + 1];
        if (u.maxpool) {
            if (p->br_act >= 0) join_branch();
            if (two_streams && any_pending()) {
                (void)hipEventRecord(p->ev_end, p->side);
                (void)hipStreamWaitEvent(main_s, p->ev_end, 0);
                clear_pending();
            }
            char* dz0 = ws + p->dz_off;
            double* ab = reinterpret_cast<double*>(ws + p->acc_off) + u.a_bwd;
            TRY(clhip_maxpool_bwd_bn_reduce(ws + dst.dy_off, ws + u.am_off, ws + u.z_off, fr + u.f_mean, fr + u.f_invstd, params + u.d.gamma_off, params + u.d.beta_off,
                                            ws + u.pg_off, ab, u.rep_bwd, p->N, u.Ho, u.Wo, u.d.cout, p->dtype, stream));
            TRY(clhip_bn_bwd_apply_acc(ws + u.pg_off, nullptr, ws + u.z_off, fr + u.f_mean, fr + u.f_invstd, params + u.d.gamma_off, params + u.d.beta_off,
                                       grads + u.d.gamma_off, grads + u.d.beta_off, dz0, nullptr, 0, u.M, u.d.cout, 0, ab, u.rep_bwd, p->dtype, stream));
            if (!(plan_skip() & 4))
                TRY(clhip_conv_wgrad(ws + src.y_off, dz0, grads + u.d.w_off, ws + u.wg_own, p->N, u.H, u.W, u.cin_pad, u.d.cin, u.d.cout, u.d.ksize, u.d.stride,
                                     u.d.pad, p->dtype, stream));
            continue;
        }
        void* dres = (u.d.res >= 0 && !u.pre_res) ? ws + p->acts[u.d.res].dy_off : nullptr;
        const bool pair_b = pair_on && u.pair >= 0 && u.d.ksize == 1 && u.pair == i - 1 && u.pair >= unit_lo;
        char* dz = ws + (two_streams ? p->dz_offs[k] : (pair_b ? p->dz_off2 : p->dz_off));
        if (br_on && u.branch >= 0 && p->bfork_ev[u.branch] != nullptr) {
            const int slot = u.branch;
            (void)hipStreamWaitEvent(p->br, p->bfork_ev[slot], 0);
            p->bfork_ev[slot] = nullptr;
            if (p->wg_pending[k]) { (void)hipStreamWaitEvent(p->br, p->ev_wg[k], 0); p->wg_pending[k] = false; }
            if (p->br_act >= 0) join_branch();
            TRY(clhip_bn_bwd_acc(ws + dst.dy_off, ws + dst.y_off, ws + u.z_off, fr + u.f_mean, fr + u.f_invstd, params + u.d.gamma_off,
                                 grads + u.d.gamma_off, grads + u.d.beta_off, dz, nullptr, 0, u.M, u.d.cout, 0,
                                 reinterpret_cast<double*>(ws + p->acc_off) + u.a_bwd, u.rep_bwd, p->dtype, p->br));
            TRY(clhip_conv_dgrad(dz, sh + u.sh_dg, ws + src.dy_off, u.dx_acc, p->N, u.H, u.W, u.cin_pad, u.d.cout, u.d.ksize, u.d.stride, u.d.pad, p->dtype, p->br));
            (void)hipEventRecord(p->ev_bjoin[slot], p->br);
            p->br_act = u.d.src; p->br_slot = slot;
            TRY(clhip_conv_wgrad(ws + src.y_off, dz, grads + u.d.w_off, ws + p->wg_off2, p->N, u.H, u.W, u.cin_pad, u.d.cin, u.d.cout,
                                 u.d.ksize, u.d.stride, u.d.pad, p->dtype, p->br));
            (void)hipEventRecord(p->ev_wg[k], p->br);
            p->wg_pending[k] = true;
            br_used = true;
            continue;
        }
        if (p->br_act >= 0 && i + 1 == p->br_act) join_branch();
        if (u.pre_res) dz = ws + p->units[u.d.res - 1].dzr_off;
        if (u.no_bn) dz = ws + u.dzr_off;
        const char* in = u.raw_src ? ws + p->units[u.d.src - 1].z_off : ws + src.y_off;
        if (two_streams && p->wg_pending[k]) {
            (void)hipStreamWaitEvent(main_s, p->ev_wg[k], 0);
            p->wg_pending[k] = false;
        }
        static const bool mask_from_y = clhip_cfg("BN_MASK_FROM_Y") != nullptr;
        const double wg_flops = 2.0 * (double)u.M * u.d.ksize * u.d.ksize * u.d.cin * u.d.cout;
        const bool on_side = two_streams && p->side_ok && wg_flops >= 1.0e9;
        static const bool ev_in_launch = clhip_cfg("EVENT_RECORD") == nullptr;
        const bool hook = on_side && ev_in_launch && !u.no_bn && u.rep_bwd > 0 && !u.has_dzr;
        if (hook) clhip_bn_set_stop_event(p->ev_dz[k]);
        const bool both = !on_side && u.d.src != 0 && !u.raw_src && !(p->br_act >= 0 && u.d.src == p->br_act) &&
                          clhip_conv_dgrad_wgrad_supported(p->N, u.H, u.W, u.cin_pad, u.d.cin, u.d.cout, u.d.ksize, u.d.stride, u.d.pad, p->dtype) &&
                          clhip_conv_wgrad_ws_bytes(p->N, u.H, u.W, u.cin_pad, u.d.cin, u.d.cout, u.d.ksize, u.d.stride, u.d.pad, p->dtype) > 0;
        const bool lazy_in = u.lazy_from >= 0 && p->lazy_live[u.lazy_from];
        const bool bn_grad_ok = both && lazy_grad_on && u.d.cout >= lazy_grad_minc && !u.no_bn && !u.pre_res && !u.has_dzr && u.rep_bwd > 0 && p->bwd_sums_ready[i] &&
                                u.relu && !mask_from_y && u.cin_pad == u.d.cin &&                                 clhip_conv_bn_input_supported(p->N, u.H, u.W, u.cin_pad, u.d.cout, u.d.ksize, u.d.stride, u.d.pad, p->dtype);
        const bool stale = p->mask_stale[i] != 0;
        const bool bn_grad = bn_grad_ok && (dres == nullptr ? true : (u.mask_off != 0 && lazy_res_on && !stale));
        if (u.no_bn || bn_grad) {
        } else if (((plan_skip() & 2) || ((plan_skip() & 8) && u.d.ksize == 1 && !u.relu)) && u.rep_bwd > 0) {
        } else if (u.rep_bwd > 0 && p->bwd_sums_ready[i]) {
            const bool zmask = u.relu && dres == nullptr && !mask_from_y;
            const bool bits = !zmask && u.relu && u.mask_off != 0 && !mask_from_y && !stale;
            TRY(clhip_bn_bwd_apply_acc(ws + dst.dy_off, zmask ? nullptr : (bits ? ws + u.mask_off : ws + dst.y_off), ws + u.z_off, fr + u.f_mean, fr + u.f_invstd,
                                       params + u.d.gamma_off, params + u.d.beta_off, grads + u.d.gamma_off, grads + u.d.beta_off, dz, dres, u.dres_acc, u.M,
                                       u.d.cout, zmask ? 2 : (bits ? 3 : (u.relu ? 1 : 0)), reinterpret_cast<double*>(ws + p->acc_off) + u.a_bwd, u.rep_bwd,
                                       p->dtype, stream));
        } else if (u.rep_bwd > 0 && u.relu && dres == nullptr && !mask_from_y) {
            TRY(clhip_bn_bwd_acc_zmask(ws + dst.dy_off, ws + u.z_off, fr + u.f_mean, fr + u.f_invstd, params + u.d.gamma_off, params + u.d.beta_off,
                                       grads + u.d.gamma_off, grads + u.d.beta_off, dz, u.M, u.d.cout,
                                       reinterpret_cast<double*>(ws + p->acc_off) + u.a_bwd, u.rep_bwd, p->dtype, stream));
        } else if (u.rep_bwd > 0) {
            const bool bits = u.relu && u.mask_off != 0 && !mask_from_y && !stale;
            TRY(clhip_bn_bwd_acc(ws + dst.dy_off, bits ? ws + u.mask_off : ws + dst.y_off, ws + u.z_off, fr + u.f_mean, fr + u.f_invstd, params + u.d.gamma_off,
                                 grads + u.d.gamma_off, grads + u.d.beta_off, dz, dres, u.dres_acc, u.M, u.d.cout, bits ? 3 : (int)u.relu,
                                 reinterpret_cast<double*>(ws + p->acc_off) + u.a_bwd, u.rep_bwd, p->dtype, stream));
        } else {
            TRY(clhip_bn_bwd(ws + dst.dy_off, ws + dst.y_off, ws + u.z_off, fr + u.f_mean, fr + u.f_invstd, params + u.d.gamma_off,
                             grads + u.d.gamma_off, grads + u.d.beta_off, dz, dres, u.dres_acc, u.M, u.d.cout, u.relu,
                             fr + p->f_bnws, p->dtype, stream));
        }
        if (u.has_dzr && !u.no_bn) TRY(clhip_add_inplace(dz, ws + u.dzr_off, u.M * u.d.cout, p->dtype, stream));
        bool dz_event_recorded = false;
        if (br_on && u.joins >= 0 && !u.pre_res && dres != nullptr) {
            if (hook && clhip_bn_pending_stop_event() == nullptr) p->bfork_ev[u.joins] = p->ev_dz[k];
            else {
                if (on_side) { clhip_bn_set_stop_event(nullptr); (void)hipEventRecord(p->ev_dz[k], main_s); dz_event_recorded = true; p->bfork_ev[u.joins] = p->ev_dz[k]; }
                else { (void)hipEventRecord(p->ev_bfork[u.joins], main_s); p->bfork_ev[u.joins] = p->ev_bfork[u.joins]; }
            }
        }
        void* wg_stream = stream;
        if (on_side) {
            if (!dz_event_recorded && (!hook || clhip_bn_pending_stop_event() != nullptr)) {
                clhip_bn_set_stop_event(nullptr);
                (void)hipEventRecord(p->ev_dz[k], main_s);
            }
            (void)hipStreamWaitEvent(p->side, p->ev_dz[k], 0);
            wg_stream = p->side;
        } else if (two_streams && any_pending() &&
                   (clhip_cfg("WGRAD_ALWAYS_QUEUE") != nullptr ||
                    clhip_conv_wgrad_ws_bytes(p->N, u.H, u.W, u.cin_pad, u.d.cin, u.d.cout, u.d.ksize, u.d.stride, u.d.pad, p->dtype) > 0)) {
            (void)hipEventRecord(p->ev_end, p->side);
            (void)hipStreamWaitEvent(main_s, p->ev_end, 0);
            clear_pending();
        }
        if (defer_side) clhip_wgrad_defer_pause(!on_side);
        if (bn_grad) {
            const Unit* prod = u.fuse_src_bn ? &p->units[u.d.src - 1] : nullptr;
            clhip_bn_grad bg;
            bg.dy = ws + dst.dy_off; bg.z = ws + u.z_off; bg.sums = reinterpret_cast<double*>(ws + p->acc_off) + u.a_bwd; bg.replicas = u.rep_bwd;
            bg.mean = fr + u.f_mean; bg.invstd = fr + u.f_invstd; bg.gamma = params + u.d.gamma_off; bg.beta = params + u.d.beta_off;
            bg.dgamma = grads + u.d.gamma_off; bg.dbeta = grads + u.d.beta_off;
            bg.relu_mask = dres != nullptr ? ws + u.mask_off : nullptr; bg.dres = dres; bg.dres_accumulate = u.dres_acc;
            const Unit* la = lazy_in ? &p->units[u.lazy_from] : nullptr;
            TRY(clhip_conv_dgrad_wgrad_bn_grad(la ? ws + la->z_off : in, la ? fr + la->f_scale : nullptr, &bg, sh + u.sh_dg, ws + src.dy_off, u.dx_acc,
                                               grads + u.d.w_off, ws + u.wg_own, prod ? ws + prod->z_off : nullptr, (prod && prod->relu) ? ws + src.y_off : nullptr,
                                               prod ? fr + prod->f_mean : nullptr, prod ? fr + prod->f_invstd : nullptr,
                                               prod ? reinterpret_cast<double*>(ws + p->acc_off) + prod->a_bwd : nullptr, prod ? prod->rep_bwd : 1, p->N, u.H, u.W,
                                               u.cin_pad, u.d.cin, u.d.cout, u.d.ksize, u.d.stride, u.d.pad, p->dtype, stream));
            if (prod) p->bwd_sums_ready[u.d.src - 1] = 1;
            continue;
        }
        if (both && u.lazy_from >= 0 && p->lazy_live[u.lazy_from]) {
            const Unit& a = p->units[u.lazy_from];
            const bool red = u.fuse_src_bn;
            TRY(clhip_conv_dgrad_wgrad_bn_input(ws + a.z_off, fr + a.f_scale, dz, sh + u.sh_dg, ws + src.dy_off, u.dx_acc, grads + u.d.w_off, ws + u.wg_own,
                                                red ? fr + a.f_mean : nullptr, red ? fr + a.f_invstd : nullptr,
                                                red ? reinterpret_cast<double*>(ws + p->acc_off) + a.a_bwd : nullptr, red ? a.rep_bwd : 1, p->N, u.H, u.W,
                                                u.cin_pad, u.d.cin, u.d.cout, u.d.ksize, u.d.stride, u.d.pad, p->dtype, stream));
            if (red) p->bwd_sums_ready[u.lazy_from] = 1;
            continue;
        }
        if (u.lazy_from >= 0) TRY(materialise(u.lazy_from));
        if (both) {
            const Unit* prod = u.fuse_src_bn ? &p->units[u.d.src - 1] : nullptr;
            TRY(clhip_conv_dgrad_wgrad(in, dz, sh + u.sh_dg, ws + src.dy_off, u.dx_acc, grads + u.d.w_off, ws + u.wg_own,
                                       prod ? ws + prod->z_off : nullptr, (prod && prod->relu) ? ws + src.y_off : nullptr, prod ? fr + prod->f_mean : nullptr,
                                       prod ? fr + prod->f_invstd : nullptr, prod ? reinterpret_cast<double*>(ws + p->acc_off) + prod->a_bwd : nullptr,
                                       prod ? prod->rep_bwd : 1, p->N, u.H, u.W, u.cin_pad, u.d.cin, u.d.cout, u.d.ksize, u.d.stride, u.d.pad, p->dtype, stream));
            if (prod) p->bwd_sums_ready[u.d.src - 1] = 1;
            continue;
        }
        if (pair_b && u.wpair) {
        } else if (pair_on && u.pair >= 0 && u.wpair && u.d.ksize == 3 && pair_dz != nullptr) {
            const Unit& sc = p->units[u.pair];
            TRY(clhip_conv_wgrad_pair(in, dz, pair_dz, grads + u.d.w_off, grads + sc.d.w_off, ws + u.wg_own, ws + sc.wg_own, p->N, u.H, u.W, u.cin_pad, u.d.cout,
                                      p->dtype, wg_stream));
        } else if (!(plan_skip() & 4))
        TRY(clhip_conv_wgrad(in, dz, grads + u.d.w_off, ws + u.wg_own, p->N, u.H, u.W, u.cin_pad, u.d.cin, u.d.cout,
                             u.d.ksize, u.d.stride, u.d.pad, p->dtype, wg_stream));
        if (defer_side && on_side && ++side_deferred % p->defer_side == 0) TRY(clhip_wgrad_defer_flush(p->side, false));
        if (on_side) {
            (void)hipEventRecord(p->ev_wg[k], p->side);
            p->wg_pending[k] = true;
        }
        if (p->br_act >= 0 && u.d.src == p->br_act && !u.raw_src) join_branch();
        if (u.raw_src) {
            TRY(clhip_conv_dgrad(dz, sh + u.sh_dg, ws + p->units[u.d.src - 1].dzr_off, 0, p->N, u.H, u.W, u.cin_pad, u.d.cout,
                                 u.d.ksize, u.d.stride, u.d.pad, p->dtype, stream));
        } else if (u.d.src != 0 && u.fuse_src_bn) {
            const Unit& prod = p->units[u.d.src - 1];
            const bool pz = prod.relu && prod.d.res < 0 && !mask_from_y, pb = prod.relu && prod.mask_off != 0 && !mask_from_y && !p->mask_stale[u.d.src - 1];
            TRY(clhip_conv_dgrad_bn_reduce_ex(dz, sh + u.sh_dg, ws + src.dy_off, u.dx_acc, ws + prod.z_off, prod.relu ? ws + src.y_off : nullptr,
                                              pb ? ws + prod.mask_off : nullptr, pz ? params + prod.d.gamma_off : nullptr, pz ? params + prod.d.beta_off : nullptr,
                                              fr + prod.f_mean, fr + prod.f_invstd, reinterpret_cast<double*>(ws + p->acc_off) + prod.a_bwd, prod.rep_bwd,
                                              p->N, u.H, u.W, u.cin_pad, u.d.cout, u.d.ksize, u.d.stride, u.d.pad, p->dtype, stream));
            p->bwd_sums_ready[u.d.src - 1] = 1;
        } else if (pair_b) {
            pair_dz = dz;
        } else if (pair_on && u.pair >= 0 && u.d.ksize == 3 && pair_dz != nullptr) {
            static const bool pfb_off = clhip_cfg("PAIR_BN_FUSE") != nullptr && atoi(clhip_cfg("PAIR_BN_FUSE")) == 0;
            if (u.pair_fuse_bn && !pfb_off) {
                const Unit& prod = p->units[u.d.src - 1];
                TRY(clhip_conv_dgrad_pair_bn_reduce(dz, sh + u.sh_pk, pair_dz, ws + src.dy_off, u.pair_acc, ws + prod.z_off, prod.relu ? ws + src.y_off : nullptr,
                                                    fr + prod.f_mean, fr + prod.f_invstd, reinterpret_cast<double*>(ws + p->acc_off) + prod.a_bwd, prod.rep_bwd, p->N, u.H, u.W,
                                                    u.cin_pad, u.d.cout, p->dtype, stream));
                p->bwd_sums_ready[u.d.src - 1] = 1;
            } else
            TRY(clhip_conv_dgrad_pair(dz, sh + u.sh_pk, pair_dz, ws + src.dy_off, u.pair_acc, p->N, u.H, u.W, u.cin_pad, u.d.cout, p->dtype, stream));
            pair_dz = nullptr;
        } else if (u.d.src != 0) {
            TRY(clhip_conv_dgrad(dz, sh + u.sh_dg, ws + src.dy_off, u.dx_acc, p->N, u.H, u.W, u.cin_pad, u.d.cout,
                                 u.d.ksize, u.d.stride, u.d.pad, p->dtype, stream));
        }
    }
    if (p->defer_reduce) { TRY(clhip_wgrad_defer_flush(main_s, true)); defer_guard.on = false; }
    if (defer_side) { clhip_wgrad_defer_pause(false); TRY(clhip_wgrad_defer_flush(p->side, true)); defer_guard.on = false; }
    if (br_used) {
        (void)hipEventRecord(p->ev_br_end, p->br);
        (void)hipStreamWaitEvent(main_s, p->ev_br_end, 0);
        p->br_act = -1;
    }
    for (int q = 0; q < clhip_plan::kMaxBranch && br_on; ++q) p->bfork_ev[q] = nullptr;
    if (two_streams && any_pending()) {
        (void)hipEventRecord(p->ev_end, p->side);
        (void)hipStreamWaitEvent(main_s, p->ev_end, 0);
        clear_pending();
    }
    return CLHIP_OK;
}

extern "C" int clhip_plan_read_act(clhip_plan* p, const void* workspace, int idx, int which, float* out_nchw, void* stream) {
    CLHIP_CHECK_ARG(p && workspace && out_nchw && idx >= 0 && idx < (int)p->acts.size() && which >= 0 && which <= 2);
    CLHIP_CHECK_ARG(!(idx == 0 && which != 0));
    if (which == 1 && idx >= 1 && p->units[idx - 1].maxpool) {
        clhip_set_error("clhip_plan_read_act: activation %d is the max-pooled stem output; its pre-pool z has another shape", idx);
        return CLHIP_EINVAL;
    }
    const char* ws = static_cast<const char*>(workspace);
    const Act& a = p->acts[idx];
    if (which == 0 && idx >= 1 && p->lazy_live[idx - 1]) {
        const Unit& ua = p->units[idx - 1];
        char* wsm = static_cast<char*>(const_cast<void*>(workspace));
        float* fr = reinterpret_cast<float*>(wsm + p->f_base);
        if (int e = clhip_bn_apply(wsm + ua.z_off, fr + ua.f_scale, fr + ua.f_shift, nullptr, wsm + a.y_off, ua.M, ua.d.cout, 1, p->dtype, stream)) return e;
        p->lazy_live[idx - 1] = 0;
    }
    if (which <= 1 && idx >= 1 && p->stage_skipped[idx - 1]) {
        clhip_set_error("clhip_plan_read_act: activation %d lies inside a run of blocks the eval forward executed as one launch (stage.hip) and was never written; "
                        "clhip_config(\"STAGE_EVAL\", \"0\") keeps one launch per unit", idx);
        return CLHIP_EINVAL;
    }
    if (which == 0 && idx >= 1 && p->eval_unwritten[idx - 1]) {
        const Unit& ua = p->units[idx - 1];
        if (p->params_dev == nullptr || p->bn_stats_dev == nullptr) { clhip_set_error("clhip_plan_read_act: activation %d was not written by the eval forward (EVAL_LAZY) and the plan has no parameter pointers to rebuild it from", idx); return CLHIP_EINVAL; }
        char* wsm = static_cast<char*>(const_cast<void*>(workspace));
        const float* params = p->params_dev; const float* bn_stats = p->bn_stats_dev;
        const void* res_e = ua.d.res >= 0 ? wsm + p->acts[ua.d.res].y_off : nullptr;
        if (int e = clhip_bn_apply_eval(wsm + ua.z_off, params + ua.d.gamma_off, params + ua.d.beta_off, bn_stats + ua.d.rm_off, bn_stats + ua.d.rv_off, kBnEps, res_e,
                                        wsm + a.y_off, ua.M, ua.d.cout, ua.relu, p->dtype, stream)) return e;
        p->eval_unwritten[idx - 1] = 0;
    }
// ... 4 lines not shown
```

### libcontinual_amd/model/backbone/resnet.py

```python
import math
import os
import weakref

import torch
import torch.nn as nn

from ... import _lib
from ..._lib import call, require_gpu

__all__ = ["HipResNet", "_Scratch", "_ScratchMixin", "cifar_resnet20", "cifar_resnet32", "cifar_resnet32_V2", "resnet18", "resnet34", "resnet32_V2",
           "CosineLinear", "SplitCosineLinear"]


def _dtype_code(dtype):
    if dtype is None:
        dtype = os.environ.get("CLHIP_DTYPE", "bf16")
    if dtype in ("bf16", torch.bfloat16, _lib.BF16):
        return _lib.BF16
    if dtype in ("f32", "fp32", "float32", torch.float32):
        return _lib.F32
    raise ValueError(f"unsupported compute dtype {dtype!r}")


class _U:
# ... 307 lines not shown
        dp = torch.Tensor.data_ptr
        return (self._flat.data_ptr(), self._stats.data_ptr(), tuple(map(dp, self._params)),
                tuple(dp(m._buffers[n]) for m, n in self._stat_holders()))

    def _stat_holders(self):
        h = self.__dict__.get("_stat_holder_cache")
        if h is None:
            mods = dict(self.named_modules())
            h = [(mods[nm.rsplit(".", 1)[0]], nm.rsplit(".", 1)[1]) for nm, _, _ in self._stat_layout]
            self.__dict__["_stat_holder_cache"] = h
        return h

    def flat_parameters(self):
        dev = self._params[0].device
        self._ensure_flat(dev)
        if self._gflat is None or self._gflat.device != dev:
            self._gflat = torch.zeros(self._nflat, device=dev, dtype=torch.float32)
        return self._flat, self._gflat

    def _grad_view(self, i):
        nm, shp, o, is_conv = self._layout[i]
        return self._view(self._gflat, shp, o, is_conv)

    def _grad_views(self):
        c = self.__dict__.get("_grad_view_cache")
        if c is None or c[0] is not self._gflat:
            c = (self._gflat, [self._grad_view(i) for i in range(len(self._params))])
            self.__dict__["_grad_view_cache"] = c
        return c[1]

    def grads_attached(self):
        c = self.__dict__.get("_grad_view_cache")
        if c is None or c[0] is not self._gflat:
            return False
        views = c[1]
        return all(p.grad is views[i] for i, p in enumerate(self._params) if p.requires_grad)

    def attach_grads(self):
        views = self._grad_views()
        for i, p in enumerate(self._params):
            if p.requires_grad and p.grad is not views[i]:
                g = views[i]
                if p.grad is not None and p.grad.data_ptr() != g.data_ptr():
                    g.copy_(p.grad)
                p.grad = g

    def begin_grad_write(self):
        _, g = self.flat_parameters()
        if all(p.grad is None for p in self._params):
            if not getattr(self, "_gflat_zeroed", False):
                g.zero_()
        self._gflat_zeroed = False
        return g

    def _plan_for(self, x):
        N, Cin, H, W = x.shape
        key = (N, H, W, self._dtype)
        ent = self._handle.plans.get(key)
        if ent is None:
            descs = (_lib.UnitDesc * len(self._units))()
            offs = {nm: o for nm, shp, o, c in self._layout}
            soffs = {nm: o for nm, shp, o in self._stat_layout}
            for i, u in enumerate(self._units):
                d = descs[i]
                d.cin, d.cout, d.ksize, d.stride, d.pad = u.cin, u.cout, u.k, u.stride, u.pad
                d.src, d.res, d.relu = u.src, u.res, int(u.relu) | u.flags
                d.w_off = offs[u.conv + ".weight"]
                if u.bn is not None:
                    d.gamma_off, d.beta_off = offs[u.bn + ".weight"], offs[u.bn + ".bias"]
                    d.rm_off, d.rv_off = soffs[u.bn + ".running_mean"], soffs[u.bn + ".running_var"]
            L = _lib.lib()
            p = L.clhip_plan_create_ex(descs, len(self._units), N, H, W, Cin, self._dtype, self._pool_win)
            if not p:
                raise _lib.ClhipError("clhip_plan_create failed: " + L.clhip_last_error().decode())
            ent = (p, (int(L.clhip_plan_workspace_bytes(p)), int(L.clhip_plan_shadow_bytes(p)), int(L.clhip_plan_feat_dim(p))))
            self._handle.plans[key] = ent
        return ent

    def _prep_weights(self, plan, shadow_bytes, dev):
        if self._shadow is None or self._shadow.device != dev or self._shadow.numel() < shadow_bytes:
            self._shadow = torch.empty(shadow_bytes, device=dev, dtype=torch.uint8)
            self._shadow_version = None
        ver = (self._flat._version, self._flat.data_ptr())
        if self._shadow_version != ver:
            call("clhip_plan_prep_weights", plan, self._flat.data_ptr(), self._shadow.data_ptr(),
                 torch.cuda.current_stream().cuda_stream)
            self._shadow_version = ver

    def compute_dtype(self, dtype):
        import contextlib

        @contextlib.contextmanager
        def scope():
            old, new = self._dtype, _dtype_code(dtype)
            if new != old:
                self._dtype, self._shadow_version = new, None
            try:
                yield self
            finally:
                if new != old:
                    self._dtype, self._shadow_version = old, None
        return scope()

    def mark_params_modified(self):
        self._shadow_version = None

    def _forward_impl(self, x, state):
        plan, ws, training = state["plan"], state["ws"], state["training"]
        feat = torch.empty(x.shape[0], state["feat_dim"], device=x.device, dtype=torch.float32)
        call("clhip_plan_forward_ex", plan, x.data_ptr(), self._flat.data_ptr(), self._stats.data_ptr(), self._shadow.data_ptr(),
             ws.data_ptr(), feat.data_ptr(), int(state.get("mode", training)), self._nbt.data_ptr() if training else None,
             torch.cuda.current_stream().cuda_stream)
        return feat

    def _backward_impl(self, dfeat, state):
        if state["gen"] != self._generation:
            raise _lib.ClhipError("backward through a backbone forward whose saved activations were overwritten by a "
                                  "later forward of the same module")
        if not state["training"]:
            raise _lib.ClhipError("backward through an eval-mode (running-stat BatchNorm) forward is not supported")
        dfeat = dfeat.contiguous().float()
        g = self.begin_grad_write()
        st = torch.cuda.current_stream().cuda_stream
        hook = self._grad_segment_hook
        if hook is None:
            call("clhip_plan_backward", state["plan"], dfeat.data_ptr(), self._flat.data_ptr(), self._shadow.data_ptr(),
                 state["ws"].data_ptr(), g.data_ptr(), st)
        else:
            hi = len(self._units)
            for lo in self._grad_segment_cuts + [0]:
                call("clhip_plan_backward_range", state["plan"], dfeat.data_ptr(), self._flat.data_ptr(), self._shadow.data_ptr(),
                     state["ws"].data_ptr(), g.data_ptr(), hi, lo, st)
                end = self._nflat if hi == len(self._units) else self._unit_off[hi]
                hook(self, self._unit_off[lo], end)
                hi = lo
        self.attach_grads()

    def takes_stage_launches(self, x):
        if x.dim() != 4:
            return False
        ent = self._handle.plans.get((x.shape[0], x.shape[2], x.shape[3], self._dtype))
        if ent is None:
            return False
        L = _lib.lib()
        if int(L.clhip_plan_stage_info(ent[0], 0)) == 0:
            return False
        sw = L.clhip_config_get(b"STAGE_TRAIN")
        return int(sw) != 0 if sw not in (None, b"") else x.shape[0] > 64

    def stage_status(self):
        L = _lib.lib()
        bad = 0
        for p, _ in self._handle.plans.values():
            bad |= int(L.clhip_plan_stage_status(p))
        return bad

    def grad_cut_for_fraction(self, frac=0.5):
        for k in range(len(self._units) - 1, 0, -1):
            if self._nflat - self._unit_off[k] >= frac * self._nflat:
                return k
        return 0

    def forward(self, x):
        require_gpu(x)
        if x.dtype != torch.float32:
            x = x.float()
        x = x.contiguous()
        dev = x.device
        self._ensure_flat(dev)
        plan, (ws_bytes, sh_bytes, feat_dim) = self._plan_for(x)
        self._prep_weights(plan, sh_bytes, dev)
        if self._ws is None or self._ws.device != dev or self._ws.numel() < ws_bytes:
            self._ws = torch.empty(ws_bytes, device=dev, dtype=torch.uint8)
        self._generation += 1
        need_grad = torch.is_grad_enabled() and self._params[0].requires_grad
        state = dict(plan=plan, ws=self._ws, training=self.training, gen=self._generation, shape=tuple(x.shape), feat_dim=feat_dim)
        if self.training and not need_grad and _NoSave.depth > 0:
            state["mode"] = 2
        self._last_state = state
        if need_grad:
            self.flat_parameters()
            feats = _BackboneFn.apply(x, self._params[0], self, state)
        else:
            feats = self._forward_impl(x, state)
        if self._returns_tensor:
            return feats
        return _Feats(feats, self, state)

    def feature(self, x):
        return self.forward(x)["features"]

    def _act_dims(self, H, W):
        dims = {0: (H, W)}
        for i, u in enumerate(self._units):
            hs, ws_ = dims[u.src]
            ho, wo = (hs + 2 * u.pad - u.k) // u.stride + 1, (ws_ + 2 * u.pad - u.k) // u.stride + 1
            if u.flags & _MAXPOOL:
                ho, wo = (ho - 1) // 2 + 1, (wo - 1) // 2 + 1
            dims[i + 1] = (ho, wo)
        return dims

    def _read_act(self, state, act, which, channels):
        if state["gen"] != self._generation:
            raise _lib.ClhipError("activation requested after the workspace was reused by a later forward")
        N, _, H, W = state["shape"]
        h, w = self._act_dims(H, W)[act]
        t = torch.empty(N, channels, h, w, device=state["ws"].device, dtype=torch.float32)
        call("clhip_plan_read_act", state["plan"], state["ws"].data_ptr(), act, which, t.data_ptr(),
             torch.cuda.current_stream().cuda_stream)
        return t

    def _read_fmaps(self, state):
        fmaps = []
        for sname, _ in self._stages:
            last = max(i for i, u in enumerate(self._units) if u.conv.startswith(sname + "."))
            fmaps.append(self._read_act(state, last + 1, 0, self._units[last].cout))
        return fmaps

    def debug_read(self, act, which=0):
        c = 8 if act == 0 else self._units[act - 1].cout
        return self._read_act(self._last_state, act, which, c)

    def __deepcopy__(self, memo):
        cls = self.__class__
        new = cls.__new__(cls)
        memo[id(self)] = new
        import copy
        for k, v in self.__dict__.items():
            if k in ("_ws", "_shadow", "_gflat", "_last_state", "_stat_holder_cache", "_grad_view_cache", "_pack_sig"):
                new.__dict__[k] = None
            elif k == "_handle":
                new.__dict__[k] = _PlanHandle()
            else:
                new.__dict__[k] = copy.deepcopy(v, memo)
        new._shadow_version = None
        named = dict(new.named_parameters())
        new._params = [named[nm] for nm, *_ in new._layout]
        new._tag_params()
        _LIVE.add(new)
        return new


def cifar_resnet20(pretrained=False, **kwargs):
    return HipResNet("cifar", depth=20, dtype=kwargs.get("dtype"))


def cifar_resnet32(pretrained=False, **kwargs):
    return HipResNet("cifar", depth=32, dtype=kwargs.get("dtype"))


def cifar_resnet32_V2(pretrained=False, **kwargs):
    return HipResNet("preact", depth=32, dtype=kwargs.get("dtype"))


def resnet32_V2(pretrained=False, **kwargs):
    return HipResNet("modified", layers=[5, 5, 5], dtype=kwargs.get("dtype"))


def stem_for(args):
    assert args is not None, "you should pass args to resnet"
    ds = args["dataset"]
    if "cifar" in ds or "5-datasets" in ds:
        return "cifar"
    if "imagenet" in ds:
        return "imagenet7" if args["init_cls_num"] == args["inc_cls_num"] else "imagenet3"
    raise NotImplementedError(f"dataset {ds!r}: the reference ResNet builds no stem for it (resnet.py:133-149)")


def _imagenet_style(layers, kwargs):
    stem = stem_for(kwargs.get("args"))
    if kwargs.get("pretrained"):
        raise NotImplementedError
    return HipResNet("imagenet_style", layers=layers, dtype=kwargs.get("dtype"), stem=stem)


def resnet18(pretrained=False, progress=True, **kwargs):
    return _imagenet_style([2, 2, 2, 2], dict(kwargs, pretrained=pretrained))


def resnet34(pretrained=False, progress=True, **kwargs):
    return _imagenet_style([3, 4, 6, 3], dict(kwargs, pretrained=pretrained))


class _Scratch:

    def __deepcopy__(self, memo):
        return _Scratch()

    def __getstate__(self):
        return {}


class _ScratchMixin:
    @property
    def last_scores(self):
        return self._scratch.scores

    @property
    def last_features(self):
        return self._scratch.features


class CosineLinear(_ScratchMixin, nn.Module):

    def __init__(self, in_features, out_features, sigma=True):
        super().__init__()
        self.in_features, self.out_features = in_features, out_features
        self._scratch = _Scratch()
        self.weight = nn.Parameter(torch.empty(out_features, in_features))
        if sigma:
            self.sigma = nn.Parameter(torch.empty(1))
        else:
# ... 42 lines not shown
```

### libcontinual_amd/ops.py

```python
import torch

from . import _lib
from ._lib import call, require_gpu

_NULL = None
UNIT_GRAD_PTRS = set()


def _st():
    return torch.cuda.current_stream().cuda_stream


def _ptr(t):
    return t.data_ptr() if t is not None else None


def _dev(*ts):
    d = None
    for t in ts:
        if t is None:
            continue
        require_gpu(t)
        if d is None:
            d = t.device
# ... 224 lines not shown
    def forward(ctx, scores, labels, num_old, K, margin, weight):
        scores = _f32c(scores)
        B, O = scores.shape
        labels = labels.to(device=scores.device, dtype=torch.int64).contiguous()
        loss = torch.empty(1, device=scores.device, dtype=torch.float32)
        ds = torch.empty_like(scores)
        hard = torch.empty(1, device=scores.device, dtype=torch.int32)
        call("clhip_margin_rank_loss", _ptr(scores), _ptr(labels), B, O, int(num_old), int(K), float(margin), float(weight),
             _ptr(loss), 0, _ptr(ds), 0, _ptr(hard), _st())
        ctx.save_for_backward(ds)
        return loss.view(())

    @staticmethod
    def backward(ctx, gout):
        (ds,) = ctx.saved_tensors
        gout = _f32c(gout.reshape(1))
        out = torch.empty_like(ds)
        call("clhip_scale_dev", _ptr(ds), _ptr(out), ds.numel(), 1.0, _ptr(gout), _st())
        return out, None, None, None, None, None


def margin_rank_loss(scores, labels, num_old, K, margin, weight=1.0):
    return _MarginRankFn.apply(scores, labels, num_old, K, margin, weight)


def ewc_penalty(p, ref, fisher, weight, loss_out, accumulate):
    _dev(p, ref, fisher, loss_out)
    call("clhip_ewc_penalty", _ptr(p), _ptr(ref), _ptr(fisher), p.numel(), float(weight), _ptr(loss_out), int(accumulate), _st())


def ewc_grad(p, ref, fisher, g, weight, dev_scale=None):
    _dev(p, ref, fisher, g, dev_scale)
    call("clhip_ewc_grad", _ptr(p), _ptr(ref), _ptr(fisher), _ptr(g), p.numel(), float(weight), _ptr(dev_scale), _st())


def _ptr_array(ts):
    import ctypes as C
    return (C.c_void_p * len(ts))(*[(t.data_ptr() if t is not None else None) for t in ts])


def ewc_penalty_multi(segs, weight, loss_out, accumulate):
    import ctypes as C
    for p, r, f in segs:
        _dev(p, r, f)
    _dev(loss_out)
    n = (C.c_int64 * len(segs))(*[p.numel() for p, _, _ in segs])
    call("clhip_ewc_penalty_multi", len(segs), _ptr_array([s[0] for s in segs]), _ptr_array([s[1] for s in segs]), _ptr_array([s[2] for s in segs]), n,
         float(weight), _ptr(loss_out), int(accumulate), _st())


def ewc_grad_multi(segs, weight, dev_scale=None):
    import ctypes as C
    for p, r, f, g in segs:
        _dev(p, r, f, g)
    n = (C.c_int64 * len(segs))(*[s[0].numel() for s in segs])
    call("clhip_ewc_grad_multi", len(segs), _ptr_array([s[0] for s in segs]), _ptr_array([s[1] for s in segs]), _ptr_array([s[2] for s in segs]),
         _ptr_array([s[3] for s in segs]), n, float(weight), _ptr(dev_scale), _st())


def fisher_accum(fisher, g, scale):
    _dev(fisher, g)
    call("clhip_fisher_accum", _ptr(fisher), _ptr(g), fisher.numel(), float(scale), _st())


def fisher_merge(new_f, old_f, alpha):
    _dev(new_f, old_f)
    call("clhip_fisher_merge", _ptr(new_f), _ptr(old_f), old_f.numel(), float(alpha), _st())


def sgd_step(p, g, mom, lr, momentum=0.0, weight_decay=0.0, grad_scale=1.0, ewc_ref=None, ewc_fisher=None, ewc_weight=0.0):
    _dev(p, g, mom, ewc_ref, ewc_fisher)
    call("clhip_sgd_step", _ptr(p), _ptr(g), _ptr(mom), p.numel(), float(lr), float(momentum), float(weight_decay),
         float(grad_scale), _ptr(ewc_ref), _ptr(ewc_fisher), float(ewc_weight), _st())


def sgd_step_multi(items, lr, momentum=0.0, weight_decay=0.0, grad_scale=1.0, zero_mask=0):
    import ctypes as C
    for p, g, m in items:
        _dev(p, g, m)
    n = (C.c_int64 * len(items))(*[it[0].numel() for it in items])
    moms = _ptr_array([it[2] for it in items]) if momentum != 0 else None
    call("clhip_sgd_step_multi_zero", len(items), _ptr_array([it[0] for it in items]), _ptr_array([it[1] for it in items]), moms, n, float(lr), float(momentum),
         float(weight_decay), float(grad_scale), int(zero_mask), _st())


def adam_step(p, g, m, v, lr, beta1, beta2, eps, weight_decay, grad_scale, step):
    _dev(p, g, m, v)
    call("clhip_adam_step", _ptr(p), _ptr(g), _ptr(m), _ptr(v), p.numel(), float(lr), float(beta1), float(beta2), float(eps),
         float(weight_decay), float(grad_scale), int(step), _st())


def sq_norm(g, out, accumulate=False):
    _dev(g, out)
    call("clhip_sq_norm", _ptr(g), g.numel(), _ptr(out), int(accumulate), _st())


def scale_(g, s):
    _dev(g)
    call("clhip_scale", _ptr(g), g.numel(), float(s), _st())


def l2_normalize_rows(x):
    x = _f32c(x)
    out = torch.empty_like(x)
    call("clhip_l2_normalize_rows", _ptr(x), _ptr(out), x.shape[0], x.shape[1], _st())
    return out


def ncm_classify(feats, means):
    feats, means = _f32c(feats), _f32c(means)
    pred = torch.empty(feats.shape[0], device=feats.device, dtype=torch.int64)
    call("clhip_ncm_classify", _ptr(feats), _ptr(means), feats.shape[0], means.shape[0], feats.shape[1], _ptr(pred), _st())
    return pred


def herding_select(feats_normed, m):
    f = _f32c(feats_normed)
    n, D = f.shape
    m = min(int(m), n)
    chosen = torch.empty(m, device=f.device, dtype=torch.int32)
    ws = torch.empty(2 * D + n, device=f.device, dtype=torch.float32)
    call("clhip_herding_select", _ptr(f), n, D, m, _ptr(chosen), _ptr(ws), _st())
    return chosen


def herding_select_classes(feats_normed, counts, m):
    f = _f32c(feats_normed)
    N, D = f.shape
    counts = [int(c) for c in counts]
    assert sum(counts) == N and len(counts) > 0
    offs = [0]
    for c in counts:
        offs.append(offs[-1] + c)
    offsets = torch.tensor(offs, dtype=torch.int32, device=f.device)
    chosen = torch.empty(len(counts), int(m), device=f.device, dtype=torch.int32)
    ws = torch.empty(2 * D * len(counts) + N, device=f.device, dtype=torch.float32)
    call("clhip_herding_select_batched", _ptr(f), _ptr(offsets), len(counts), max(counts), D, int(m), _ptr(chosen), _ptr(ws), _st())
    return [chosen[i, : min(int(m), c)] for i, c in enumerate(counts)]


def clip_grad_norm_(params, max_norm, eps=1e-6):
    grads = [p.grad for p in params if p.grad is not None]
    if not grads:
        return None
    _dev(*grads)
    sq = torch.zeros(1, device=grads[0].device, dtype=torch.float32)
    flat = []
    for g in grads:
        if g.dtype != torch.float32 or not g.is_contiguous():
            raise _lib.ClhipError("clip_grad_norm_: gradients must be contiguous fp32")
        call("clhip_sq_norm", _ptr(g), g.numel(), _ptr(sq), 1, _st())
        flat.append(g)
    norm = sq.sqrt()
    coef = (max_norm / (norm + eps)).clamp(max=1.0)
    for g in flat:
        call("clhip_scale_dev", _ptr(g), _ptr(g), g.numel(), 1.0, _ptr(coef), _st())
    return norm


_SIDE_STREAMS = {}


def _env_unset(name):
    return __import__("os").environ.get(name) is None


# ... 46 lines not shown
```

### libcontinual_amd/optim.py

```python
import torch

from . import ops
from ._lib import require_gpu


def _owner_of(p):
    ref = getattr(p, "_clhip_owner", None)
    return ref() if ref is not None else None


def _tag_backbones(params):
    owners = {}
    for p in params:
        o = _owner_of(p)
        if o is not None:
            owners.setdefault(id(o), (o, []))[1].append(p)
    return owners


class _FusedBase(torch.optim.Optimizer):
    grad_scale = 1.0
    capture_safe = False
    zero_grads_in_step = False

# ... 26 lines not shown
    @staticmethod
    def _dense(p):
        if p.is_contiguous():
            return p.data.view(-1)
        if p.dim() == 4 and p.is_contiguous(memory_format=torch.channels_last):
            return p.data.permute(0, 2, 3, 1).reshape(-1)
        raise RuntimeError("parameter is neither contiguous nor channels_last")

    @staticmethod
    def _dense_like(p, g):
        if g.is_contiguous() and p.is_contiguous():
            return g.view(-1)
        if g.dim() == 4 and g.is_contiguous(memory_format=torch.channels_last) and p.is_contiguous(memory_format=torch.channels_last):
            return g.permute(0, 2, 3, 1).reshape(-1)
        if p.dim() == 4 and p.is_contiguous(memory_format=torch.channels_last):
            return g.contiguous(memory_format=torch.channels_last).permute(0, 2, 3, 1).reshape(-1)
        return g.contiguous().view(-1)


def _dp_plan(o):
    d = getattr(o, "_dp_shard", None)
    if d is None:
        return [(o._flat, o._gflat, "")], None
    o._dp_shard = None
    n = o._flat.numel()
    parts = []
    if d["hi"] > d["lo"]:
        parts.append((o._flat[d["lo"]:d["hi"]], d["grad"], "_shard"))
    if d["prefix"] < n:
        parts.append((o._flat[d["prefix"]:], o._gflat[d["prefix"]:], "_tail"))
    return parts, d


class SGD(_FusedBase):
    capture_safe = True

    def __init__(self, params, lr=1e-3, momentum=0.0, dampening=0, weight_decay=0.0, nesterov=False):
        if dampening != 0 or nesterov:
            raise NotImplementedError("dampening / nesterov are not used by the reference configs")
        super().__init__(params, dict(lr=lr, momentum=momentum, weight_decay=weight_decay))

    @torch.no_grad()
    def step(self, closure=None):
        batches = {}
        for group in self.param_groups:
            lr, mom, wd = group["lr"], group["momentum"], group["weight_decay"]
            whole, rest = self._split(group)
            self._check_unconsumed_shards(rest)
            entry = batches.setdefault((lr, mom, wd), [[], [], 0, []])
            items, after = entry[0], entry[1]
            for o in whole:
                require_gpu(o._flat)
                st = self.state[o._params[0]]
                parts, shard = _dp_plan(o)
                if self.zero_grads_in_step and shard is None and len(parts) == 1 and len(items) < 8:
                    entry[2] |= 1 << len(items)
                    entry[3].append(o)
                for flat, gflat, sfx in parts:
                    buf = None
                    if mom != 0:
                        buf = st.get("flat_momentum" + sfx)
                        if buf is None or buf.data_ptr() == 0 or buf.numel() != flat.numel() or buf.device != flat.device:
                            buf = torch.zeros_like(flat)
                            st["flat_momentum" + sfx] = buf
                    items.append((flat, gflat, buf))
                after.append((o, shard))
            for p in rest:
                require_gpu(p)
                st = self.state[p]
                pd = self._dense(p)
                gd = self._dense_like(p, p.grad)
                buf = None
                if mom != 0:
                    buf = st.get("momentum_buffer")
                    if buf is None:
                        buf = torch.zeros(pd.numel(), device=p.device, dtype=torch.float32)
                        st["momentum_buffer"] = buf
                items.append((pd, gd, buf))
                o = _owner_of(p)
                if o is not None:
                    after.append((o, None))
        for (lr, mom, wd), (items, after, zero_mask, zeroed) in batches.items():
            same_dev = len({it[0].device for it in items}) <= 1
            if (len(items) >= 2 or zero_mask) and same_dev:
                for k in range(0, len(items), 8):
                    ops.sgd_step_multi(items[k:k + 8], lr, mom, wd, self.grad_scale, zero_mask if k == 0 else 0)
                for o in zeroed:
                    o._gflat_zeroed = True
            else:
                for pd, gd, buf in items:
                    ops.sgd_step(pd, gd, buf, lr, mom, wd, self.grad_scale)
            for o, shard in after:
                if shard is not None:
                    o._dp_shard = shard
                    shard["reducer"].gather_params(o)
                    o._dp_shard = None
                o.mark_params_modified()
        return None


class Adam(_FusedBase):
    def __init__(self, params, lr=1e-3, betas=(0.9, 0.999), eps=1e-8, weight_decay=0.0, amsgrad=False):
        if amsgrad:
            raise NotImplementedError
        super().__init__(params, dict(lr=lr, betas=betas, eps=eps, weight_decay=weight_decay))

    @torch.no_grad()
    def step(self, closure=None):
        for group in self.param_groups:
            lr, (b1, b2), eps, wd = group["lr"], group["betas"], group["eps"], group["weight_decay"]
            whole, rest = self._split(group)
            self._check_unconsumed_shards(rest)
            items, publish = [], []
            for o in whole:
                parts, shard = _dp_plan(o)
                items += [((o._params[0], sfx), flat, gflat, o) for flat, gflat, sfx in parts]
                if shard is not None:
                    publish.append((o, shard))
            items += [((p, ""), self._dense(p), self._dense_like(p, p.grad), _owner_of(p)) for p in rest]
            for (key, sfx), pd, gd, o in items:
                require_gpu(pd)
                st = self.state[key]
                if "step" + sfx not in st or st["exp_avg" + sfx].numel() != pd.numel():
                    st["step" + sfx] = 0
                    st["exp_avg" + sfx] = torch.zeros(pd.numel(), device=pd.device, dtype=torch.float32)
                    st["exp_avg_sq" + sfx] = torch.zeros(pd.numel(), device=pd.device, dtype=torch.float32)
                st["step" + sfx] += 1
                ops.adam_step(pd, gd, st["exp_avg" + sfx], st["exp_avg_sq" + sfx], lr, b1, b2, eps, wd, self.grad_scale, st["step" + sfx])
                if o is not None:
                    o.mark_params_modified()
            for o, shard in publish:
                o._dp_shard = shard
                shard["reducer"].gather_params(o)
                o._dp_shard = None
                o.mark_params_modified()
        return None
```

Before: 126,400 images/sec.

## Fuse SGD update with bf16 shadow weight prep in one kernel

Adds a plan-aware SGD kernel that updates the flat fp32 conv parameters and momentum and writes the bf16 forward, dgrad and paired-packed shadow weights in the same pass. Extra parameter tensors such as BN and FC are handled by additional blocks of the same launch. This removes the separate weight-prep kernel and its re-read of the parameters before the next forward pass. The diff also adds a separate wgrad workspace for small layers so the main-stream and side-stream wgrad no longer share a buffer. In exchange there is more complex shadow-version bookkeeping in Python, which risks stale shadow weights if a parameter changes outside this path.

```diff
diff --git a/include/clhip.h b/include/clhip.h
--- a/include/clhip.h
+++ b/include/clhip.h
@@ -125,6 +125,10 @@
 long long clhip_plan_stage_info(const clhip_plan*, int what);
 int clhip_plan_stage_trace(clhip_plan*, unsigned long long* out24);
 int clhip_plan_prep_weights(clhip_plan*, const float* params, void* shadow, void* stream);
+int clhip_plan_sgd_prep_supported(const clhip_plan*);
+int clhip_plan_sgd_prep(clhip_plan*, float* params, float* grads, float* momentum_buf , int64_t n_flat, void* shadow, int n_extra, float* const* xp,
+                        float* const* xg, float* const* xm , const int64_t* xn, float lr, float momentum, float weight_decay, float grad_scale,
+                        unsigned zero_grad_mask, void* stream);
 int clhip_plan_forward(clhip_plan*, const float* x, const float* params, float* bn_stats, const void* shadow,
                        void* workspace, float* feat, int training, void* stream);
 int clhip_plan_forward_ex(clhip_plan*, const float* x, const float* params, float* bn_stats, const void* shadow,
diff --git a/libcontinual_amd/_lib.py b/libcontinual_amd/_lib.py
--- a/libcontinual_amd/_lib.py
+++ b/libcontinual_amd/_lib.py
@@ -112,6 +112,8 @@
     "clhip_plan_stage_info": (C.c_longlong, [_p, _i]),
     "clhip_plan_stage_trace": (_i, [_p, _p]),
     "clhip_plan_prep_weights": (_i, [_p, _p, _p, _p]),
+    "clhip_plan_sgd_prep_supported": (_i, [_p]),
+    "clhip_plan_sgd_prep": (_i, [_p, _p, _p, _p, _l, _p, _i, _p, _p, _p, _p, _f, _f, _f, _f, C.c_uint, _p]),
     "clhip_plan_forward": (_i, [_p, _p, _p, _p, _p, _p, _p, _i, _p]),
     "clhip_plan_forward_ex": (_i, [_p, _p, _p, _p, _p, _p, _p, _i, _p, _p]),
     "clhip_plan_backward": (_i, [_p, _p, _p, _p, _p, _p, _p]),
diff --git a/libcontinual_amd/csrc/api.hip b/libcontinual_amd/csrc/api.hip
--- a/libcontinual_amd/csrc/api.hip
+++ b/libcontinual_amd/csrc/api.hip
@@ -24,10 +24,10 @@
 namespace {
 const char* const kKeys[] = {
     "ATTN_GENERIC", "ATTN_BWD", "BN_FUSE", "BN_FUSE_MAX_M", "BN_MASK_BITS", "BN_MASK_FROM_Y", "BN_PARTIALS", "CE_ROWS", "CE_ONE_WG", "LINEAR_BWD_SPLIT", "CONV3G", "CONV4", "CONV_V1",
-    "GEMM_NO_SPLIT", "GEMM_TAIL", "NO_CONV16", "NO_CONV3", "NO_PARITY_DGRAD", "NO_SHORTCUT", "NO_STEM", "PREP_NARROW", "WGRAD4",
+    "GEMM_NO_SPLIT", "GEMM_TAIL", "NO_CONV16", "NO_CONV3", "NO_PARITY_DGRAD", "NO_SHORTCUT", "NO_STEM", "PREP_NARROW", "SGD_PREP", "WGRAD_MAIN_JOIN", "WGRAD4",
     "WGRAD_NO_TR", "WGRAD2_ATOMIC", "WGRAD_DEFER", "WGRAD_DEFER_SIDE", "BWD_FUSED", "WGRAD_STREAM", "BRANCH_STREAM", "WGRAD_ALWAYS_QUEUE", "SIDE_PRIO", "EVENT_FLAGS", "EVENT_RECORD", "CONV5", "CONV6", "WGRAD16_PARTS", "WGRAD32_IPG", "WGRAD64_IPG", "WGRAD64_IPI2", "CONV64", "CONV64_BM", "CONV64_FWD", "CONV6_PAIR", "CONV7", "CONV7_TPW", "WGRAD7", "FWD7", "PAIR_BN_FUSE", "POOL_BN_FUSE", "BN_INPUT", "BN_INPUT_WT", "BN_RES_INPUT", "BN_GRAD", "BN_GRAD_MINC", "BN_GRAD_RES", "CONV6_DEBUG", "BN_ONEPASS", "WGRAD5", "WGRAD32",
     "BN_ACC_CPT", "BN_BWD_ITERS", "CONV3_CFG", "CONV4_CFG", "CONV4_GRID", "GEMM_GROUP_M", "GEMM_MT", "IGEMM_TILE",
-    "SHORTCUT_MIN_PIXELS", "STEM_GRID", "STEM_WGRAD_GRID", "WGRAD4_MIN_STEPS", "WGRAD4_MIN_TOTAL", "WGRAD_NET_GFLOP", "WGRAD_TARGET",
+    "SHORTCUT_MIN_PIXELS", "STEM_GRID", "STEM_WGRAD_GRID", "WGRAD4_MIN_STEPS", "WGRAD4_MIN_TOTAL", "WGRAD_NET_GFLOP", "WGRAD_SIDE_GFLOP", "WGRAD_TARGET",
     "CONV5_MIN_TILES", "CONV5_GRID", "CONV64_MAX_W", "CONV64_MAX_M", "CONV8", "CONV8_MIN_TILES", "DZ_BUFFERS", "CONV8_GRID", "CONV8_OPT", "CONV8_BNR", "CONV9", "PLAN_SKIP", "WT_DEBUG", "EVAL_LAZY", "GEMM_SPLITK", "STREAM_PROBE", "STAGE_EVAL", "STAGE_TRAIN", "STAGE_TRAIN_BWD", "STAGE_TRACE", "STAGE_ENTRY", "STAGE_ENTRY_BWD", "STAGE_POOL", "STAGE_XCH3",
     "CONV3_DEBUG", "WGRAD_DEBUG", "CONV4_FORCE_CFG", "CONV4_ENABLE", "CONV4_DEBUG", "CONV4_TRACE", "WGRAD4_TRACE", "CONV6_TRACE", "CONV8_TRACE", "CONV9_TRACE",
 };
diff --git a/libcontinual_amd/csrc/common.h b/libcontinual_amd/csrc/common.h
--- a/libcontinual_amd/csrc/common.h
+++ b/libcontinual_amd/csrc/common.h
@@ -45,6 +45,17 @@
 __device__ __forceinline__ uint32_t pack_bf16x2(float lo, float hi) {
     f32x2_t v = {lo, hi};
     return __builtin_bit_cast(uint32_t, __builtin_convertvector(v, bf16x2_t));
+}
+
+template <bool MOM>
+__device__ __forceinline__ float sgd_update(float pv, float g, float& mv, float lr, float momentum, float wd, float gscale) {
+    float d = g * gscale;
+    d = fmaf(wd, pv, d);
+    if (MOM) {
+        mv = fmaf(momentum, mv, d);
+        d = mv;
+    }
+    return fmaf(-lr, d, pv);
 }
 
 template <typename T> struct Elem;
diff --git a/libcontinual_amd/csrc/elementwise.hip b/libcontinual_amd/csrc/elementwise.hip
--- a/libcontinual_amd/csrc/elementwise.hip
+++ b/libcontinual_amd/csrc/elementwise.hip
@@ -113,15 +113,9 @@
     const SgdSeg& e = t.s[u];
     const long long stride = (long long)e.blocks * 256;
     for (long long i = (long long)(blockIdx.x - e.first_block) * 256 + threadIdx.x; i < e.n; i += stride) {
-        float pv = e.p[i];
-        float d = e.g[i] * gscale;
-        d = fmaf(wd, pv, d);
-        if (MOM) {
-            float b = fmaf(momentum, e.m[i], d);
-            e.m[i] = b;
-            d = b;
-        }
-        e.p[i] = fmaf(-lr, d, pv);
+        float mv = MOM ? e.m[i] : 0.f;
+        e.p[i] = sgd_update<MOM>(e.p[i], e.g[i], mv, lr, momentum, wd, gscale);
+        if (MOM) e.m[i] = mv;
         if (e.zero) e.g[i] = 0.f;
     }
 }
diff --git a/libcontinual_amd/csrc/plan.hip b/libcontinual_amd/csrc/plan.hip
--- a/libcontinual_amd/csrc/plan.hip
+++ b/libcontinual_amd/csrc/plan.hip
@@ -130,6 +130,10 @@
     long long st_fwd_launches = 0, st_bwd_launches = 0;
     int feat_dim;
     bool side_ok;
+    double side_layer_flops;
+    size_t wg_main;
+    bool main_join;
+    bool sgd_prep;
     int pool_win;
 };
 
@@ -281,6 +285,9 @@
     {
         const double net_flops = 1.0e9 * (clhip_cfg("WGRAD_NET_GFLOP") ? atof(clhip_cfg("WGRAD_NET_GFLOP")) : 4.0);
         p->side_ok = false;
+        p->side_layer_flops = 1.0e9 * (clhip_cfg("WGRAD_SIDE_GFLOP") ? atof(clhip_cfg("WGRAD_SIDE_GFLOP")) : 1.0);
+        p->main_join = clhip_cfg("WGRAD_MAIN_JOIN") != nullptr && atoi(clhip_cfg("WGRAD_MAIN_JOIN")) != 0;
+        p->sgd_prep = !(clhip_cfg("SGD_PREP") != nullptr && atoi(clhip_cfg("SGD_PREP")) == 0);
         for (const Unit& u : p->units)
             if (2.0 * (double)u.M * u.d.ksize * u.d.ksize * u.d.cin * u.d.cout >= net_flops) p->side_ok = true;
     }
@@ -308,6 +315,14 @@
         }
     }
     p->wg_off2 = off; off = align_up(off + max_wg2);
+    p->wg_main = p->wg_off;
+    if (p->side_ok && !p->main_join) {
+        size_t max_main = 0;
+        for (const Unit& u : p->units)
+            if (2.0 * (double)u.M * u.d.ksize * u.d.ksize * u.d.cin * u.d.cout < p->side_layer_flops)
+                max_main = std::max(max_main, clhip_conv_wgrad_ws_bytes(N, u.H, u.W, u.cin_pad, u.d.cin, u.d.cout, u.d.ksize, u.d.stride, u.d.pad, dtype));
+        p->wg_main = off; off = align_up(off + max_main);
+    }
     p->f_base = off;
     nfloat = (nfloat + 63) / 64 * 64;
     p->f_part = nfloat; nfloat += (max_part + 63) / 64 * 64;
@@ -718,6 +733,167 @@
         }
     }
 }
+
+constexpr int kSgdExtra = 7;
+struct SgdPrepEntry { int64_t w_off, wf_off, wd_off, wp_off; int wp_tap0, K, taps, Creal, Cpad, tail_n; };
+struct SgdPrepExtra { float* p; float* g; float* m; long long n; unsigned first_block, blocks; int zero; };
+struct SgdPrepTable { int n, n_extra; unsigned tail_first, extra_first; unsigned first[kPrepMax]; SgdPrepEntry e[kPrepMax]; SgdPrepExtra x[kSgdExtra]; };
+static_assert(sizeof(SgdPrepTable) + 64 <= 4096, "the table travels in the kernel arguments");
+
+template <bool MOM>
+__global__ __launch_bounds__(256) void sgd_prep_kernel(float* __restrict__ params, float* __restrict__ grads, float* __restrict__ mom, char* __restrict__ shadow,
+                                                       SgdPrepTable t, float lr, float momentum, float wd, float gscale, int zero) {
+    __shared__ float tile[64][65];
+    if (blockIdx.x >= t.extra_first) {
+        int s = 0;
+        while (s + 1 < t.n_extra && blockIdx.x >= t.x[s + 1].first_block) ++s;
+        const SgdPrepExtra& e = t.x[s];
+        const long long stride = (long long)e.blocks * 256;
+        for (long long i = (long long)(blockIdx.x - e.first_block) * 256 + threadIdx.x; i < e.n; i += stride) {
+            float mv = MOM ? e.m[i] : 0.f;
+            e.p[i] = sgd_update<MOM>(e.p[i], e.g[i], mv, lr, momentum, wd, gscale);
+            if (MOM) e.m[i] = mv;
+            if (e.zero) e.g[i] = 0.f;
+        }
+        return;
+    }
+    if (blockIdx.x >= t.tail_first) {
+        const SgdPrepEntry& d = t.e[blockIdx.x - t.tail_first];
+        const int64_t base = d.w_off + (int64_t)d.K * d.taps * d.Creal;
+        for (int i = threadIdx.x; i < d.tail_n; i += 256) {
+            float mv = MOM ? mom[base + i] : 0.f;
+            params[base + i] = sgd_update<MOM>(params[base + i], grads[base + i], mv, lr, momentum, wd, gscale);
+            if (MOM) mom[base + i] = mv;
+            if (zero) grads[base + i] = 0.f;
+        }
+        return;
+    }
+    const int l = threadIdx.x & 63;
+    const bool le = l < t.n && t.first[l < kPrepMax ? l : 0] <= blockIdx.x;
+    const int u = __builtin_amdgcn_readfirstlane(__popcll(__ballot(le)) - 1);
+    const SgdPrepEntry& d = t.e[u];
+    const int kb = (d.K + 63) / 64, cb = (d.Cpad + 63) / 64;
+    int r = blockIdx.x - t.first[u];
+    const int c0 = (r % cb) * 64; r /= cb;
+    const int k0 = (r % kb) * 64;
+    const int tap = r / kb;
+    const int tx = (threadIdx.x & 15) * 4, ty = threadIdx.x >> 4;
+    const bool vec = (d.Creal & 3) == 0;
+    bf16_t* wf = reinterpret_cast<bf16_t*>(shadow + d.wf_off);
+#pragma unroll
+    for (int i = 0; i < 4; ++i) {
+        const int kk = ty + 16 * i, k = k0 + kk, c = c0 + tx;
+        float v[4] = {0.f, 0.f, 0.f, 0.f};
+        if (k < d.K && c < d.Cpad) {
+            const int64_t idx = d.w_off + ((int64_t)k * d.taps + tap) * d.Creal + c;
+            if (vec && c < d.Creal) {
+                const float4 pv = *reinterpret_cast<const float4*>(params + idx), gv = *reinterpret_cast<const float4*>(grads + idx);
+                float4 mv = MOM ? *reinterpret_cast<const float4*>(mom + idx) : make_float4(0.f, 0.f, 0.f, 0.f);
+                v[0] = sgd_update<MOM>(pv.x, gv.x, mv.x, lr, momentum, wd, gscale);
+                v[1] = sgd_update<MOM>(pv.y, gv.y, mv.y, lr, momentum, wd, gscale);
+                v[2] = sgd_update<MOM>(pv.z, gv.z, mv.z, lr, momentum, wd, gscale);
+                v[3] = sgd_update<MOM>(pv.w, gv.w, mv.w, lr, momentum, wd, gscale);
+                *reinterpret_cast<float4*>(params + idx) = make_float4(v[0], v[1], v[2], v[3]);
+                if (MOM) *reinterpret_cast<float4*>(mom + idx) = mv;
+                if (zero) *reinterpret_cast<float4*>(grads + idx) = make_float4(0.f, 0.f, 0.f, 0.f);
+            } else if (!vec) {
+#pragma unroll
+                for (int e = 0; e < 4; ++e)
+                    if (c + e < d.Creal) {
+                        float mv = MOM ? mom[idx + e] : 0.f;
+                        v[e] = sgd_update<MOM>(params[idx + e], grads[idx + e], mv, lr, momentum, wd, gscale);
+                        params[idx + e] = v[e];
+                        if (MOM) mom[idx + e] = mv;
+                        if (zero) grads[idx + e] = 0.f;
+                    }
+            }
+            *reinterpret_cast<uint2*>(wf + ((size_t)k * d.taps + tap) * d.Cpad + c) = make_uint2(pack_bf16x2(v[0], v[1]), pack_bf16x2(v[2], v[3]));
+        }
+#pragma unroll
+        for (int e = 0; e < 4; ++e) tile[kk][tx + e] = v[e];
+    }
+    if (d.wd_off < 0) return;
+    __syncthreads();
+    bf16_t* wdg = reinterpret_cast<bf16_t*>(shadow + d.wd_off);
+#pragma unroll
+    for (int i = 0; i < 4; ++i) {
+        const int cc = ty + 16 * i, c = c0 + cc, k = k0 + tx;
+        if (c < d.Cpad && k < d.K) {
+            const uint2 v = make_uint2(pack_bf16x2(tile[tx][cc], tile[tx + 1][cc]), pack_bf16x2(tile[tx + 2][cc], tile[tx + 3][cc]));
+            *reinterpret_cast<uint2*>(wdg + ((size_t)c * d.taps + tap) * d.K + k) = v;
+            if (d.wp_off >= 0) *reinterpret_cast<uint2*>(reinterpret_cast<bf16_t*>(shadow + d.wp_off) + packed_index(c, d.wp_tap0 + tap, k, d.K, d.Cpad)) = v;
+        }
+    }
+}
+}
+
+static bool prep_wide_ok(const clhip_plan* p, size_t lo, size_t hi) {
+    static const bool no_wide = clhip_cfg("PREP_NARROW") != nullptr;
+    bool wide = p->dtype == CLHIP_BF16 && !no_wide;
+    for (size_t j = lo; j < p->units.size() && j < hi; ++j)
+        wide = wide && p->units[j].d.cout % 4 == 0 && p->units[j].cin_pad % 4 == 0 && p->units[j].sh_fwd % 8 == 0 && p->units[j].sh_dg % 8 == 0;
+    return wide;
+}
+
+extern "C" int clhip_plan_sgd_prep_supported(const clhip_plan* p) {
+    if (p == nullptr || !p->sgd_prep || p->units.size() > (size_t)kPrepMax || !prep_wide_ok(p, 0, p->units.size())) return 0;
+    int64_t end = 0;
+    for (size_t i = 0; i < p->units.size(); ++i) {
+        const Unit& u = p->units[i];
+        if (u.d.w_off % 4 != 0 || (i == 0 ? u.d.w_off != 0 : u.d.w_off < end) || u.d.w_off - end > (1 << 20)) return 0;
+        end = u.d.w_off + (int64_t)u.d.cout * u.d.ksize * u.d.ksize * u.d.cin;
+        if (u.pair >= 0 && (u.d.ksize == 3 ? u.sh_pk : p->units[u.pair].sh_pk) % 8 != 0) return 0;
+    }
+    return 1;
+}
+
+extern "C" int clhip_plan_sgd_prep(clhip_plan* p, float* params, float* grads, float* momentum_buf, int64_t n_flat, void* shadow, int n_extra, float* const* xp,
+                                   float* const* xg, float* const* xm, const int64_t* xn, float lr, float momentum, float weight_decay, float grad_scale,
+                                   unsigned zero_grad_mask, void* stream) {
+    CLHIP_CHECK_ARG(p && params && grads && shadow && n_extra >= 0 && n_extra <= kSgdExtra);
+    CLHIP_CHECK_ARG(momentum == 0.f || momentum_buf != nullptr);
+    CLHIP_CHECK_ARG(n_extra == 0 || (xp && xg && xn && (momentum == 0.f || xm)));
+    if (!clhip_plan_sgd_prep_supported(p)) { clhip_set_error("clhip_plan_sgd_prep: not supported for this plan (clhip_plan_sgd_prep_supported)"); return CLHIP_EINVAL; }
+    const Unit& lu = p->units.back();
+    const int64_t last_end = lu.d.w_off + (int64_t)lu.d.cout * lu.d.ksize * lu.d.ksize * lu.d.cin;
+    CLHIP_CHECK_ARG(n_flat >= last_end && n_flat - last_end <= (1 << 20));
+    SgdPrepTable t;
+    t.n = 0; t.n_extra = 0;
+    unsigned blocks = 0;
+    for (size_t i = 0; i < p->units.size(); ++i) {
+        const Unit& u = p->units[i];
+        SgdPrepEntry& e = t.e[t.n];
+        e.w_off = u.d.w_off; e.wf_off = (int64_t)u.sh_fwd; e.wd_off = u.d.src != 0 ? (int64_t)u.sh_dg : -1;
+        e.wp_off = -1; e.wp_tap0 = 0;
+        if (u.pair >= 0) {
+            const bool owner = u.d.ksize == 3;
+            e.wp_off = (int64_t)(owner ? u.sh_pk : p->units[u.pair].sh_pk);
+            e.wp_tap0 = owner ? 0 : 9;
+        }
+        e.K = u.d.cout; e.taps = u.d.ksize * u.d.ksize; e.Creal = u.d.cin; e.Cpad = u.cin_pad;
+        const int64_t next = i + 1 < p->units.size() ? p->units[i + 1].d.w_off : n_flat;
+        e.tail_n = (int)(next - (e.w_off + (int64_t)e.K * e.taps * e.Creal));
+        t.first[t.n++] = blocks;
+        blocks += (unsigned)(e.taps * ((e.K + 63) / 64) * ((e.Cpad + 63) / 64));
+    }
+    t.tail_first = blocks;
+    blocks += (unsigned)t.n;
+    t.extra_first = blocks;
+    for (int k = 0; k < n_extra; ++k) {
+        CLHIP_CHECK_ARG(xn[k] >= 0 && (xn[k] == 0 || (xp[k] && xg[k] && (momentum == 0.f || xm[k]))));
+        if (xn[k] == 0) continue;
+        SgdPrepExtra& e = t.x[t.n_extra++];
+        e.p = xp[k]; e.g = xg[k]; e.m = momentum != 0.f ? xm[k] : nullptr; e.n = xn[k]; e.zero = (zero_grad_mask >> (k + 1)) & 1u;
+        e.first_block = blocks;
+        e.blocks = (unsigned)std::min<int64_t>((xn[k] + 1023) / 1024, 1024);
+        blocks += e.blocks;
+    }
+    const int zero = (int)(zero_grad_mask & 1u);
+    char* sh = static_cast<char*>(shadow);
+    if (momentum != 0.f) hipLaunchKernelGGL(sgd_prep_kernel<true>, dim3(blocks), dim3(256), 0, (hipStream_t)stream, params, grads, momentum_buf, sh, t, lr, momentum, weight_decay, grad_scale, zero);
+    else hipLaunchKernelGGL(sgd_prep_kernel<false>, dim3(blocks), dim3(256), 0, (hipStream_t)stream, params, grads, momentum_buf, sh, t, lr, momentum, weight_decay, grad_scale, zero);
+    CLHIP_LAUNCH_CHECK();
+    return CLHIP_OK;
 }
 
 extern "C" int clhip_plan_prep_weights(clhip_plan* p, const float* params, void* shadow, void* stream) {
@@ -728,10 +904,7 @@
         PrepTable t;
         t.n = 0;
         unsigned blocks = 0;
-        bool wide = p->dtype == CLHIP_BF16;
-        static const bool no_wide = clhip_cfg("PREP_NARROW") != nullptr;
-        for (size_t j = i; j < p->units.size() && j < i + kPrepMax; ++j)
-            wide = wide && !no_wide && p->units[j].d.cout % 4 == 0 && p->units[j].cin_pad % 4 == 0 && p->units[j].sh_fwd % 8 == 0 && p->units[j].sh_dg % 8 == 0;
+        const bool wide = prep_wide_ok(p, i, i + kPrepMax);
         const int tb = wide ? 64 : 32;
         for (; i < p->units.size() && t.n < kPrepMax; ++i) {
             const Unit& u = p->units[i];
@@ -1274,7 +1447,8 @@
         }
         static const bool mask_from_y = clhip_cfg("BN_MASK_FROM_Y") != nullptr;
         const double wg_flops = 2.0 * (double)u.M * u.d.ksize * u.d.ksize * u.d.cin * u.d.cout;
-        const bool on_side = two_streams && p->side_ok && wg_flops >= 1.0e9;
+        const bool on_side = two_streams && p->side_ok && wg_flops >= p->side_layer_flops;
+        char* wg_ws = ws + ((two_streams && p->side_ok && !on_side && !p->main_join && !p->defer_reduce && p->defer_side == 0) ? p->wg_main : u.wg_own);
         static const bool ev_in_launch = clhip_cfg("EVENT_RECORD") == nullptr;
         const bool hook = on_side && ev_in_launch && !u.no_bn && u.rep_bwd > 0 && !u.has_dzr;
         if (hook) clhip_bn_set_stop_event(p->ev_dz[k]);
@@ -1328,7 +1502,7 @@
             wg_stream = p->side;
         } else if (two_streams && any_pending() &&
                    (clhip_cfg("WGRAD_ALWAYS_QUEUE") != nullptr ||
-                    clhip_conv_wgrad_ws_bytes(p->N, u.H, u.W, u.cin_pad, u.d.cin, u.d.cout, u.d.ksize, u.d.stride, u.d.pad, p->dtype) > 0)) {
+                    (p->main_join && clhip_conv_wgrad_ws_bytes(p->N, u.H, u.W, u.cin_pad, u.d.cin, u.d.cout, u.d.ksize, u.d.stride, u.d.pad, p->dtype) > 0))) {
             (void)hipEventRecord(p->ev_end, p->side);
             (void)hipStreamWaitEvent(main_s, p->ev_end, 0);
             clear_pending();
@@ -1343,7 +1517,7 @@
             bg.relu_mask = dres != nullptr ? ws + u.mask_off : nullptr; bg.dres = dres; bg.dres_accumulate = u.dres_acc;
             const Unit* la = lazy_in ? &p->units[u.lazy_from] : nullptr;
             TRY(clhip_conv_dgrad_wgrad_bn_grad(la ? ws + la->z_off : in, la ? fr + la->f_scale : nullptr, &bg, sh + u.sh_dg, ws + src.dy_off, u.dx_acc,
-                                               grads + u.d.w_off, ws + u.wg_own, prod ? ws + prod->z_off : nullptr, (prod && prod->relu) ? ws + src.y_off : nullptr,
+                                               grads + u.d.w_off, wg_ws, prod ? ws + prod->z_off : nullptr, (prod && prod->relu) ? ws + src.y_off : nullptr,
                                                prod ? fr + prod->f_mean : nullptr, prod ? fr + prod->f_invstd : nullptr,
                                                prod ? reinterpret_cast<double*>(ws + p->acc_off) + prod->a_bwd : nullptr, prod ? prod->rep_bwd : 1, p->N, u.H, u.W,
                                                u.cin_pad, u.d.cin, u.d.cout, u.d.ksize, u.d.stride, u.d.pad, p->dtype, stream));
@@ -1353,7 +1527,7 @@
         if (both && u.lazy_from >= 0 && p->lazy_live[u.lazy_from]) {
             const Unit& a = p->units[u.lazy_from];
             const bool red = u.fuse_src_bn;
-            TRY(clhip_conv_dgrad_wgrad_bn_input(ws + a.z_off, fr + a.f_scale, dz, sh + u.sh_dg, ws + src.dy_off, u.dx_acc, grads + u.d.w_off, ws + u.wg_own,
+            TRY(clhip_conv_dgrad_wgrad_bn_input(ws + a.z_off, fr + a.f_scale, dz, sh + u.sh_dg, ws + src.dy_off, u.dx_acc, grads + u.d.w_off, wg_ws,
                                                 red ? fr + a.f_mean : nullptr, red ? fr + a.f_invstd : nullptr,
                                                 red ? reinterpret_cast<double*>(ws + p->acc_off) + a.a_bwd : nullptr, red ? a.rep_bwd : 1, p->N, u.H, u.W,
                                                 u.cin_pad, u.d.cin, u.d.cout, u.d.ksize, u.d.stride, u.d.pad, p->dtype, stream));
@@ -1363,7 +1537,7 @@
         if (u.lazy_from >= 0) TRY(materialise(u.lazy_from));
         if (both) {
             const Unit* prod = u.fuse_src_bn ? &p->units[u.d.src - 1] : nullptr;
-            TRY(clhip_conv_dgrad_wgrad(in, dz, sh + u.sh_dg, ws + src.dy_off, u.dx_acc, grads + u.d.w_off, ws + u.wg_own,
+            TRY(clhip_conv_dgrad_wgrad(in, dz, sh + u.sh_dg, ws + src.dy_off, u.dx_acc, grads + u.d.w_off, wg_ws,
                                        prod ? ws + prod->z_off : nullptr, (prod && prod->relu) ? ws + src.y_off : nullptr, prod ? fr + prod->f_mean : nullptr,
                                        prod ? fr + prod->f_invstd : nullptr, prod ? reinterpret_cast<double*>(ws + p->acc_off) + prod->a_bwd : nullptr,
                                        prod ? prod->rep_bwd : 1, p->N, u.H, u.W, u.cin_pad, u.d.cin, u.d.cout, u.d.ksize, u.d.stride, u.d.pad, p->dtype, stream));
@@ -1373,10 +1547,10 @@
         if (pair_b && u.wpair) {
         } else if (pair_on && u.pair >= 0 && u.wpair && u.d.ksize == 3 && pair_dz != nullptr) {
             const Unit& sc = p->units[u.pair];
-            TRY(clhip_conv_wgrad_pair(in, dz, pair_dz, grads + u.d.w_off, grads + sc.d.w_off, ws + u.wg_own, ws + sc.wg_own, p->N, u.H, u.W, u.cin_pad, u.d.cout,
+            TRY(clhip_conv_wgrad_pair(in, dz, pair_dz, grads + u.d.w_off, grads + sc.d.w_off, wg_ws, wg_ws == ws + u.wg_own ? ws + sc.wg_own : wg_ws, p->N, u.H, u.W, u.cin_pad, u.d.cout,
                                       p->dtype, wg_stream));
         } else if (!(plan_skip() & 4))
-        TRY(clhip_conv_wgrad(in, dz, grads + u.d.w_off, ws + u.wg_own, p->N, u.H, u.W, u.cin_pad, u.d.cin, u.d.cout,
+        TRY(clhip_conv_wgrad(in, dz, grads + u.d.w_off, wg_ws, p->N, u.H, u.W, u.cin_pad, u.d.cin, u.d.cout,
                              u.d.ksize, u.d.stride, u.d.pad, p->dtype, wg_stream));
         if (defer_side && on_side && ++side_deferred % p->defer_side == 0) TRY(clhip_wgrad_defer_flush(p->side, false));
         if (on_side) {
diff --git a/libcontinual_amd/model/backbone/resnet.py b/libcontinual_amd/model/backbone/resnet.py
--- a/libcontinual_amd/model/backbone/resnet.py
+++ b/libcontinual_amd/model/backbone/resnet.py
@@ -413,10 +413,13 @@
             self._shadow = torch.empty(shadow_bytes, device=dev, dtype=torch.uint8)
             self._shadow_version = None
         ver = (self._flat._version, self._flat.data_ptr())
-        if self._shadow_version != ver:
+        by = self.__dict__.get("_shadow_by")
+        if self._shadow_version != ver or (by is not None and (by != plan or torch.cuda.is_current_stream_capturing() or
+                                                               self._shadow_pver != tuple(p._version for p in self._params))):
             call("clhip_plan_prep_weights", plan, self._flat.data_ptr(), self._shadow.data_ptr(),
                  torch.cuda.current_stream().cuda_stream)
             self._shadow_version = ver
+            self._shadow_by = None
 
     def compute_dtype(self, dtype):
         import contextlib
@@ -435,6 +438,23 @@
 
     def mark_params_modified(self):
         self._shadow_version = None
+
+    def fused_step_target(self):
+        st, sh = self._last_state, self._shadow
+        if st is None or sh is None or st.get("dtype") != self._dtype or sh.device != self._flat.device:
+            return None
+        ent = self._handle.plans.get((st["shape"][0], st["shape"][2], st["shape"][3], self._dtype))
+        if ent is None or ent[0] != st["plan"] or sh.numel() < ent[1][1]:
+            return None
+        ok = self._handle.__dict__.setdefault("sgd_prep_ok", {})
+        if st["plan"] not in ok:
+            ok[st["plan"]] = bool(_lib.lib().clhip_plan_sgd_prep_supported(st["plan"]))
+        return (st["plan"], sh) if ok[st["plan"]] else None
+
+    def mark_shadow_current(self, plan):
+        self._shadow_version = (self._flat._version, self._flat.data_ptr())
+        self._shadow_pver = tuple(p._version for p in self._params)
+        self._shadow_by = plan
 
     def _forward_impl(self, x, state):
         plan, ws, training = state["plan"], state["ws"], state["training"]
@@ -505,7 +525,7 @@
             self._ws = torch.empty(ws_bytes, device=dev, dtype=torch.uint8)
         self._generation += 1
         need_grad = torch.is_grad_enabled() and self._params[0].requires_grad
-        state = dict(plan=plan, ws=self._ws, training=self.training, gen=self._generation, shape=tuple(x.shape), feat_dim=feat_dim)
+        state = dict(plan=plan, ws=self._ws, training=self.training, gen=self._generation, shape=tuple(x.shape), feat_dim=feat_dim, dtype=self._dtype)
         if self.training and not need_grad and _NoSave.depth > 0:
             state["mode"] = 2
         self._last_state = state
@@ -558,7 +578,7 @@
         memo[id(self)] = new
         import copy
         for k, v in self.__dict__.items():
-            if k in ("_ws", "_shadow", "_gflat", "_last_state", "_stat_holder_cache", "_grad_view_cache", "_pack_sig"):
+            if k in ("_ws", "_shadow", "_gflat", "_last_state", "_stat_holder_cache", "_grad_view_cache", "_pack_sig", "_shadow_by"):
                 new.__dict__[k] = None
             elif k == "_handle":
                 new.__dict__[k] = _PlanHandle()
diff --git a/libcontinual_amd/ops.py b/libcontinual_amd/ops.py
--- a/libcontinual_amd/ops.py
+++ b/libcontinual_amd/ops.py
@@ -330,6 +330,18 @@
     moms = _ptr_array([it[2] for it in items]) if momentum != 0 else None
     call("clhip_sgd_step_multi_zero", len(items), _ptr_array([it[0] for it in items]), _ptr_array([it[1] for it in items]), moms, n, float(lr), float(momentum),
          float(weight_decay), float(grad_scale), int(zero_mask), _st())
+
+
+def plan_sgd_prep(plan, flat, gflat, mom, shadow, extras, lr, momentum=0.0, weight_decay=0.0, grad_scale=1.0, zero_mask=0):
+    import ctypes as C
+    _dev(flat, gflat, mom, shadow)
+    for p, g, m in extras:
+        _dev(p, g, m)
+    xn = (C.c_int64 * max(len(extras), 1))(*[it[0].numel() for it in extras])
+    xm = _ptr_array([it[2] for it in extras]) if momentum != 0 and extras else None
+    call("clhip_plan_sgd_prep", plan, _ptr(flat), _ptr(gflat), _ptr(mom) if momentum != 0 else None, flat.numel(), _ptr(shadow), len(extras),
+         _ptr_array([it[0] for it in extras]) if extras else None, _ptr_array([it[1] for it in extras]) if extras else None, xm, xn,
+         float(lr), float(momentum), float(weight_decay), float(grad_scale), int(zero_mask), _st())
 
 
 def adam_step(p, g, m, v, lr, beta1, beta2, eps, weight_decay, grad_scale, step):
diff --git a/libcontinual_amd/optim.py b/libcontinual_amd/optim.py
--- a/libcontinual_amd/optim.py
+++ b/libcontinual_amd/optim.py
@@ -132,6 +132,22 @@
                     after.append((o, None))
         for (lr, mom, wd), (items, after, zero_mask, zeroed) in batches.items():
             same_dev = len({it[0].device for it in items}) <= 1
+            fused = None
+            if same_dev and items and 1 <= len(items) <= 8 and after and after[0][1] is None and items[0][0] is after[0][0]._flat:
+                fused = after[0][0].fused_step_target()
+            if fused is not None:
+                o = after[0][0]
+                ops.plan_sgd_prep(fused[0], items[0][0], items[0][1], items[0][2], fused[1], items[1:], lr, mom, wd, self.grad_scale, zero_mask)
+                for z in zeroed:
+                    z._gflat_zeroed = True
+                for b, shard in after:
+                    if shard is not None:
+                        b._dp_shard = shard
+                        shard["reducer"].gather_params(b)
+                        b._dp_shard = None
+                    b.mark_params_modified()
+                o.mark_shadow_current(fused[0])
+                continue
             if (len(items) >= 2 or zero_mask) and same_dev:
                 for k in range(0, len(items), 8):
                     ops.sgd_step_multi(items[k:k + 8], lr, mom, wd, self.grad_scale, zero_mask if k == 0 else 0)
```

Result: no change. 127,200 images/sec, median of 6 (+0.7%).
